# xuchang116/smCounter

Hardware: AMD Instinct MI355X
Metric: loci/sec at fixed read-depth x rpb (higher is better)
Workload: dtype u8/u32 scan + f64 posterior

## Files before the change

### include/smcounter_hip.h

```cpp
#ifndef SMCOUNTER_HIP_H
#define SMCOUNTER_HIP_H

#include <stdint.h>

#ifdef __cplusplus
extern "C" {
#endif

#define SMC_ABI_VERSION 11
#define SMC_MAX_ALLELES 64

#define SMC_OK 0
#define SMC_E_ARG (-1)
#define SMC_E_HIP (-2)
#define SMC_E_NOGPU (-3)
#define SMC_E_INPUT (-4)

#define SMC_ST_OK 0
#define SMC_ST_ZERO_COVERAGE 1
#define SMC_ST_DOWNSAMPLED 0x100
#define SMC_ST_BAD_INPUT 0x200
#define SMC_ST_UNDERFLOW 0x400

#define SMC_F_LM 0x001
// ... 307 lines not shown
int smc_spike_alleles(smc_ctx* ctx, const smc_dev_aln* d_aln, int64_t n_aln, const uint32_t* d_cig, const uint8_t* d_bq, int64_t n_pairs,
                      const smc_spike_variant* d_var, const smc_spike_variant* var_host, int32_t n_var, const uint64_t* d_idents,
                      int64_t n_bc, uint64_t seed, double mismatch_thr, const int32_t* d_nm, const int32_t* d_n_indel,
                      smc_dev_aln* d_aln_out, uint8_t* d_bq_out, uint32_t* d_stats, void* stream);
typedef struct smc_spike_indel_variant {
    int32_t pos0;
    uint8_t kind;
    uint8_t ref, alt;
    uint8_t pad;
    uint16_t len;
    uint16_t lead;
    uint32_t ins_off;
    uint64_t thr;
} smc_spike_indel_variant;
int smc_spike_indels(smc_ctx* ctx, const smc_dev_aln* d_aln, int64_t n_aln, const uint32_t* d_cig, int64_t n_cig_words, const uint8_t* d_bq,
                     int64_t n_pairs, const smc_spike_indel_variant* d_var, const smc_spike_indel_variant* var_host, int32_t n_var,
                     const uint8_t* d_ins, int64_t n_ins, const uint64_t* d_idents, int64_t n_bc, uint64_t seed, double mismatch_thr,
                     const int32_t* d_nm, const int32_t* d_n_indel, int64_t cap_pairs, int64_t cap_cig, smc_dev_aln* d_aln_out,
                     uint8_t* d_bq_out, uint32_t* d_cig_out, int32_t* d_nm_out, int32_t* d_n_indel_out, uint32_t* d_stats,
                     uint64_t* d_totals, void* stream);
#define SMC_SPIKE_MAX_COPIES 64
#define SMC_SPIKE_REP_MAX_TARGETS 32
int smc_spike_alleles_reps(smc_ctx* ctx, const smc_dev_aln* d_aln, int64_t n_aln, const uint32_t* d_cig, const uint8_t* d_bq, int64_t n_pairs,
                           const smc_spike_variant* d_var, const smc_spike_variant* var_host, int32_t n_var, const uint64_t* d_idents,
                           int64_t n_bc, const uint64_t* seeds, const uint64_t* thr, int32_t n_copies, double mismatch_thr,
                           const int32_t* d_nm, const int32_t* d_n_indel, uint8_t* d_aln_out, int64_t aln_stride, uint8_t* d_bq_out,
                           int64_t bq_stride, uint32_t* d_stats, void* stream);
int smc_spike_rep_counts(smc_ctx* ctx, const uint64_t* d_cov_ident, const uint32_t* d_cov_cnt, const uint32_t* d_cov_off,
                         const uint32_t* cov_off_host, const uint32_t* d_pos1, int32_t n_var, const uint64_t* d_seeds, int32_t n_reps,
                         const uint64_t* thr, int32_t n_targets, uint32_t* d_out, void* stream);
int smc_spike_depth_counts(smc_ctx* ctx, const uint64_t* d_cov_ident, const uint32_t* d_cov_cnt, const uint32_t* d_cov_off,
                           const uint32_t* cov_off_host, const uint32_t* d_pos1, int32_t n_var, const uint64_t* d_seeds, int32_t n_reps,
                           const uint64_t* thr, int32_t n_targets, const uint64_t* depth_thr, int32_t n_fracs, uint32_t* d_out, void* stream);
#define SMC_SPIKE_PHASE_MAX_MEMBERS 8
int smc_spike_phase_counts(smc_ctx* ctx, const uint64_t* d_joint_ident, const uint32_t* d_joint_cnt, const uint32_t* d_joint_off,
                           const uint32_t* joint_off_host, const uint32_t* d_set_m, const uint32_t* set_m_host, const uint32_t* d_cnt_off,
                           const uint32_t* d_pos1, int32_t n_sets, const uint64_t* d_seeds, int32_t n_reps, const uint64_t* thr,
                           int32_t n_targets, const uint64_t* depth_thr, int32_t n_fracs, uint32_t* d_out, void* stream);
int smc_spike_indels_reps(smc_ctx* ctx, const smc_dev_aln* d_aln, int64_t n_aln, const uint32_t* d_cig, int64_t n_cig_words, const uint8_t* d_bq,
                          int64_t n_pairs, const smc_spike_indel_variant* d_var, const smc_spike_indel_variant* var_host, int32_t n_var,
                          const uint8_t* d_ins, int64_t n_ins, const uint64_t* d_idents, int64_t n_bc, const uint64_t* seeds, const uint64_t* thr,
                          int32_t n_copies, double mismatch_thr, const int32_t* d_nm, const int32_t* d_n_indel, int64_t cap_pairs,
                          int64_t cap_cig, uint8_t* d_aln_out, int64_t aln_stride, uint8_t* d_bq_out, int64_t bq_stride, uint8_t* d_cig_out,
                          int64_t cig_stride, int32_t* d_nm_out, int32_t* d_n_indel_out, uint32_t* d_stats, uint64_t* d_totals, void* stream);
int smc_spike_indel_touch(smc_ctx* ctx, const smc_dev_aln* d_aln, int64_t n_aln, const uint32_t* d_cig, int64_t n_cig_words, int64_t n_pairs,
                          const smc_spike_indel_variant* d_var, const smc_spike_indel_variant* var_host, int32_t n_var, int64_t n_bc,
                          uint32_t* d_out, void* stream);
int smc_spike_indel_counts(smc_ctx* ctx, const uint64_t* d_cov_ident, const uint32_t* d_cov_cnt, const uint32_t* d_cov_off,
                           const uint32_t* cov_off_host, const uint32_t* d_pos1, int32_t n_var, const uint64_t* d_seeds, int32_t n_reps,
                           const uint64_t* thr, int32_t n_targets, const uint64_t* depth_thr, int32_t n_fracs, uint32_t* d_out, void* stream);
int smc_spike_indel_phase_counts(smc_ctx* ctx, const uint64_t* d_joint_ident, const uint32_t* d_joint_cnt, const uint32_t* d_joint_off,
                                 const uint32_t* joint_off_host, const uint32_t* d_set_m, const uint32_t* set_m_host, const uint32_t* d_cnt_off,
                                 const uint32_t* d_pos1, int32_t n_sets, const uint64_t* d_seeds, int32_t n_reps, const uint64_t* thr,
                                 int32_t n_targets, const uint64_t* depth_thr, int32_t n_fracs, uint32_t* d_out, void* stream);
int smc_spike_read_bits(smc_ctx* ctx, const smc_dev_aln* d_aln, int64_t n_aln, const uint32_t* d_cig, int64_t n_cig_words, const uint8_t* d_bq,
                        int64_t n_pairs, const smc_dev_locus* d_loc, int64_t n_loci, int32_t start0, const smc_af_variant* d_var,
                        const smc_af_variant* var_host, int32_t n_var, uint8_t* d_out, void* stream);
int smc_spike_rpb_counts(smc_ctx* ctx, const uint64_t* d_cov_ident, const uint32_t* d_cov_off, const uint32_t* cov_off_host,
                         const uint32_t* d_rec_off, const uint32_t* rec_off_host, const uint64_t* d_rec_name, const uint8_t* d_rec_flag,
                         int64_t n_rec, const uint32_t* d_pos1, int32_t n_var, const uint64_t* d_seeds, int32_t n_reps, const uint64_t* thr,
                         int32_t n_targets, const uint64_t* read_thr, int32_t n_read_thr, uint32_t* d_out, void* stream);
int smc_read_groups_counts_frac_seeds(smc_read_groups* g, const uint64_t* seeds, int32_t n_seeds, const uint64_t* bc_thr, int32_t n_frac,
                                      uint64_t* counts);
int smc_spike_grid_counts(smc_ctx* ctx, const uint64_t* d_cov_ident, const uint32_t* d_cov_off, const uint32_t* cov_off_host,
                          const uint32_t* d_rec_off, const uint32_t* rec_off_host, const uint64_t* d_rec_name, const uint8_t* d_rec_flag,
                          int64_t n_rec, const uint32_t* d_pos1, int32_t n_var, const uint64_t* d_seeds, int32_t n_reps, const uint64_t* thr,
                          int32_t n_targets, const uint64_t* bc_thr, int32_t n_fracs, const uint64_t* d_rd_thr, const uint64_t* rd_thr_host,
                          int32_t n_read_thr, uint32_t* d_out, void* stream);
int smc_spike_indel_read_bits(smc_ctx* ctx, const smc_dev_aln* d_aln, int64_t n_aln, const uint32_t* d_cig, int64_t n_cig_words,
                              const uint8_t* d_bq, int64_t n_pairs, const smc_dev_locus* d_loc, int64_t n_loci, int32_t start0,
                              const smc_spike_indel_variant* d_var, const smc_spike_indel_variant* var_host, int32_t n_var,
                              const uint8_t* d_ins, int64_t n_ins, uint8_t* d_out, void* stream);
int smc_spike_indel_rpb_counts(smc_ctx* ctx, const uint64_t* d_cov_ident, const uint32_t* d_cov_off, const uint32_t* cov_off_host,
                               const uint32_t* d_rec_off, const uint32_t* rec_off_host, const uint64_t* d_rec_name, const uint8_t* d_rec_flag,
                               int64_t n_rec, const uint32_t* d_pos1, int32_t n_var, const uint64_t* d_seeds, int32_t n_reps,
                               const uint64_t* thr, int32_t n_targets, const uint64_t* read_thr, int32_t n_read_thr, uint32_t* d_out,
                               void* stream);
int smc_spike_phase_rpb_counts(smc_ctx* ctx, const uint64_t* d_joint_ident, const uint32_t* d_joint_off, const uint32_t* joint_off_host,
                               const uint32_t* d_set_m, const uint32_t* set_m_host, const uint32_t* d_seg_base, const uint32_t* seg_base_host,
                               const uint32_t* d_rec_off, const uint32_t* rec_off_host, const uint64_t* d_rec_name, const uint8_t* d_rec_flag,
                               int64_t n_rec, const uint32_t* d_pos1, int32_t n_sets, const uint64_t* d_seeds, int32_t n_reps,
                               const uint64_t* thr, int32_t n_targets, const uint64_t* read_thr, int32_t n_read_thr, uint32_t* d_out,
                               void* stream);

typedef struct smc_scan_locus {
    uint32_t offset;
    uint32_t alt;
} smc_scan_locus;
typedef struct smc_scan_verdict {
    double pi;
    int32_t vmt;
    uint32_t mt_verdict;
} smc_scan_verdict;
#define SMC_SCAN_NOT 0u
#define SMC_SCAN_CALLED 1u
#define SMC_SCAN_HOST 2u
#define SMC_SCAN_MT_MASK 0x3FFFFFFFu
int smc_scan_detect(smc_ctx* ctx, const smc_row* d_rows, int32_t n_copies, int64_t n_loci, const smc_scan_locus* d_listed,
                    const smc_scan_locus* listed_host, int32_t n_listed, double thr, smc_scan_verdict* d_out, uint32_t* d_host_list,
                    uint32_t* d_n_host, void* stream);
#define SMC_SCAN_ID_NONE 0xFFFFFFFFu
#define SMC_SCAN_ID_HOST 0xFFFFFFFEu
int smc_scan_detect_keys(smc_ctx* ctx, const smc_row* d_rows, int32_t n_copies, int64_t n_loci, const smc_af_variant* d_var,
                         const smc_af_variant* var_host, int32_t n_listed, const uint8_t* d_ins, int64_t n_ins, const smc_dev_aln* d_aln,
                         int64_t aln_stride, const uint32_t* d_cig, int64_t cig_stride, const uint8_t* d_bq, int64_t bq_stride, int64_t n_aln,
                         int64_t cap_pairs, const uint32_t* d_x, int64_t x_stride, const uint32_t* d_xcount, int64_t xcount_stride,
                         int64_t xcap, double thr, uint32_t* d_alt_id, smc_scan_verdict* d_out, uint32_t* d_host_list, uint32_t* d_n_host,
                         void* stream);
#define SMC_F_REPT 0x0400u
#define SMC_F_REPS 0x0800u
#define SMC_F_SL 0x1000u
#define SMC_F_OTHER_REPEAT 0x2000u
#define SMC_SCAN_FLT_DEVICE_MASK 0x3FFu
#define SMC_SCAN_FLT_NAMES_MASK 0x3FFFu
#define SMC_SCAN_FLT_HOST 0x80000000u
int smc_scan_filter(smc_ctx* ctx, const smc_row* d_rows, int32_t n_copies, int64_t n_loci, const uint32_t* d_offsets,
                    const uint32_t* offsets_host, const uint32_t* d_gate, const uint32_t* gate_host, const uint32_t* d_always,
                    const uint32_t* always_host, int32_t n_listed, uint32_t* d_out, void* stream);
int smc_plan_info(const smc_plan* plan, int32_t* n_launches, int64_t* scratch_bytes);

int smc_plan_set_timing(smc_plan* plan, int slots);
int smc_plan_kernel_ms(smc_plan* plan, float* avg_ms, int32_t* n_samples, int64_t* n_loci, int64_t* n_reads);

int smc_plan_run(smc_plan* plan, const smc_params* params, const uint32_t* meta,
                 const uint32_t* umi, const uint32_t* frag, const uint32_t* dist,
                 const uint32_t* umi_start, smc_row* rows, void* stream);
int smc_plan_run_words(smc_plan* plan, const smc_params* params, const uint32_t* words, const uint32_t* umi_start,
                       smc_row* rows, void* stream);
int smc_plan_run_words16(smc_plan* plan, const smc_params* params, const uint16_t* words16, const uint32_t* umi_start,
                         smc_row* rows, void* stream);
int smc_pack_words(smc_plan* plan, const uint32_t* meta, const uint32_t* frag, uint32_t* words, void* stream);

int smc_call_batch_host(smc_ctx* ctx, const smc_params* params, const smc_locus* loci,
                        int64_t n_loci, const uint32_t* meta, const uint32_t* umi,
                        const uint32_t* frag, const uint32_t* dist, int64_t n_slots,
                        const uint32_t* umi_start, int64_t n_umi_start, smc_row* rows_out);

int smc_wire_row_size(void);
int smc_pack_rows(smc_ctx* ctx, const smc_row* rows, int64_t n, smc_wire_row* wire, void* stream);
int smc_unpack_rows(const smc_wire_row* wire, int64_t n, smc_row* rows);

typedef struct smc_build_in {
    const smc_dev_aln* aln; const uint32_t* cig;
    const uint8_t* bq;
    const smc_dev_locus* loc; const uint8_t* refseq;
    int32_t start0, n_loci, n_bc, n_pair;
    int32_t max_depth;
    int32_t n_aln;
    const smc_dev_locus* loc_host;
} smc_build_in;
int smc_build_max_depth(void);
int smc_build_set_timing(smc_ctx* ctx, int slots);
int smc_build_kernel_ms(smc_ctx* ctx, float* avg_ms, int32_t* n_samples);
int smc_build_planes(smc_ctx* ctx, const smc_params* params, const smc_build_in* in, uint32_t slot_base, uint32_t umi_base,
                     uint32_t* words, uint32_t* meta, uint32_t* umi, uint32_t* frag, uint32_t* dist, uint32_t* umi_start,
                     uint32_t* u_gid, uint32_t* u_finc, smc_locus* loci, uint32_t* xlist, uint32_t xcap, uint32_t* counters, void* stream);

int smc_build_planes_w16(smc_ctx* ctx, const smc_params* params, const smc_build_in* in, uint32_t slot_base, uint32_t umi_base,
                         uint16_t* words16, uint32_t* umi_start, uint32_t* u_gid, uint32_t* u_finc, smc_locus* loci,
                         uint32_t* xlist, uint32_t xcap, uint32_t* counters, void* stream);

#define SMC_LISTED_MAX_LOCI 64
#define SMC_LISTED_MAX_COPIES 1024
#define SMC_LISTED_UNFLAGGED 64u
#define SMC_LISTED_SHARED_ORDER 1
#define SMC_LISTED_DENSE_LOCUS 2
typedef struct smc_listed_copy {
    const smc_dev_aln* aln; const uint32_t* cig; const uint8_t* bq; const smc_dev_locus* loc;
    int32_t n_aln, n_bc, n_pair, reserved;
} smc_listed_copy;
int smc_build_listed(smc_ctx* ctx, const smc_params* params, const smc_listed_copy* d_copies, int32_t n_copies, int32_t flags,
                     int32_t start0, int32_t n_loci, const uint8_t* d_refseq, const uint32_t* offsets, const uint32_t* caps,
                     int32_t n_listed, int32_t word_bits, uint32_t slot_base, uint32_t umi_base, void* words, uint32_t* umi_start,
                     uint32_t* u_gid, uint32_t* u_finc, smc_locus* loci, uint32_t* xlist, uint32_t xcap, uint32_t* counters,
                     void* stream);

int smc_pool_trim(smc_ctx* ctx);

int smc_mem_alloc(smc_ctx* ctx, int64_t bytes, void** out);
void smc_mem_free(smc_ctx* ctx, void* p);
int smc_mem_alloc_best(smc_ctx* ctx, int64_t bytes, int tries, void** out, float* info);
int smc_mem_write_probe(smc_ctx* ctx, void* p, int64_t bytes, float* ms);
int smc_mem_alloc_host(smc_ctx* ctx, int64_t bytes, void** out);
void smc_mem_free_host(smc_ctx* ctx, void* p);
int smc_mem_h2d(smc_ctx* ctx, void* dst_device, const void* src_host, int64_t bytes);
int smc_mem_d2h(smc_ctx* ctx, void* dst_host, const void* src_device, int64_t bytes);
int smc_device_sync(smc_ctx* ctx);

int smc_event_create(void** ev);
int smc_event_record(void* ev, void* stream);
int smc_event_elapsed_ms(void* start, void* stop, float* ms);
void smc_event_destroy(void* ev);

#ifdef __cplusplus
}
#endif
#endif
```

### smcounter_amd/_lib.py

```python
from __future__ import annotations

import ctypes
import os

from . import abi

HERE = os.path.dirname(os.path.abspath(__file__))
LIB_PATH = os.environ.get("SMC_HIP_LIB") or os.path.join(HERE, "libsmcounter_hip.so")

SYMBOLS = ("smc_abi_version", "smc_last_error", "smc_row_size", "smc_locus_size", "smc_device_count",
           "smc_create", "smc_destroy", "smc_plan_create", "smc_plan_create_dev", "smc_plan_create_dev_spec", "smc_plan_spec_ok", "smc_plan_spec_counts", "smc_plan_hint_reset", "smc_philox_marks", "smc_philox4x32_10_host", "smc_select_alignments", "smc_select_alignments_keyed", "smc_select_alignments_copies", "smc_select_alignments_reads_copies", "smc_read_groups_create", "smc_read_groups_add", "smc_read_groups_finish",
           "smc_read_groups_masks", "smc_read_groups_kept", "smc_read_groups_status", "smc_read_groups_destroy",
           "smc_read_groups_counts_frac", "smc_read_groups_masks_grid", "smc_read_groups_kept_grid", "smc_lod_table", "smc_fisher_tables", "smc_lfact_values", "smc_allele_carriers", "smc_af_rep_masks", "smc_af_rep_counts", "smc_af_depth_masks", "smc_af_depth_counts", "smc_spike_alleles", "smc_spike_indels", "smc_spike_alleles_reps", "smc_spike_rep_counts", "smc_spike_depth_counts", "smc_spike_phase_counts", "smc_spike_indels_reps", "smc_spike_indel_touch", "smc_spike_indel_counts", "smc_spike_indel_phase_counts", "smc_spike_read_bits", "smc_spike_rpb_counts", "smc_spike_indel_read_bits", "smc_spike_indel_rpb_counts", "smc_spike_phase_rpb_counts", "smc_read_groups_counts_frac_seeds", "smc_spike_grid_counts", "smc_scan_detect", "smc_scan_detect_keys", "smc_scan_filter", "smc_plan_destroy", "smc_plan_info",
           "smc_plan_run", "smc_plan_run_words", "smc_plan_run_words16", "smc_pack_words", "smc_plan_set_timing", "smc_plan_kernel_ms", "smc_call_batch_host", "smc_event_create", "smc_event_record",
           "smc_event_elapsed_ms", "smc_event_destroy", "smc_class_table", "smc_wire_row_size", "smc_pack_rows", "smc_unpack_rows",
           "smc_build_planes", "smc_build_planes_w16", "smc_build_listed", "smc_build_max_depth", "smc_build_set_timing", "smc_build_kernel_ms", "smc_mem_alloc", "smc_mem_alloc_best", "smc_mem_write_probe", "smc_mem_free", "smc_mem_h2d", "smc_mem_d2h",
           "smc_mem_alloc_host", "smc_mem_free_host", "smc_pool_trim",
           "smc_device_sync")


class SmcError(RuntimeError):
    pass


def exp_env(name: str, default=None):
    on = os.environ.get("SMC_EXPERIMENTAL", "0") not in ("", "0")
    return os.environ.get(name, default) if on else default


_LIB = None


def load(with_torch: bool = True):
    global _LIB
    if _LIB is not None:
        return _LIB
    if not os.path.exists(LIB_PATH):
        try:
            from . import build
            build.build_hip()
        except Exception as e:
            raise SmcError("HIP library missing: %s and it could not be built (%s) - run `python -c 'import "
                           "__graft_entry__ as g; g.build()'`; there is no CPU fallback" % (LIB_PATH, e))
    if with_torch:
        try:
            import torch
        except ImportError:
            pass
    L = ctypes.CDLL(LIB_PATH)
    vp, i32, i64 = ctypes.c_void_p, ctypes.c_int32, ctypes.c_int64
    L.smc_abi_version.restype = ctypes.c_int
    L.smc_last_error.restype = ctypes.c_char_p
    L.smc_row_size.restype = ctypes.c_int
    L.smc_locus_size.restype = ctypes.c_int
    L.smc_device_count.restype = ctypes.c_int
    L.smc_create.argtypes = [ctypes.c_int, ctypes.POINTER(vp)]
    L.smc_destroy.argtypes = [vp]
    L.smc_destroy.restype = None
    L.smc_plan_create.argtypes = [vp, vp, i64, ctypes.POINTER(vp)]
    L.smc_plan_create_dev.argtypes = [vp, vp, i64, vp, ctypes.POINTER(vp)]
    L.smc_plan_create_dev_spec.argtypes = [vp, ctypes.POINTER(abi.SmcParams), vp, i64, vp, ctypes.POINTER(vp)]
    L.smc_plan_spec_ok.argtypes = [vp, ctypes.POINTER(ctypes.c_int)]
    L.smc_plan_spec_counts.argtypes = [vp, ctypes.POINTER(i64), ctypes.POINTER(i64), ctypes.POINTER(i64)]
    L.smc_plan_hint_reset.argtypes = [vp]
    L.smc_philox_marks.argtypes = [vp, ctypes.POINTER(abi.SmcParams), vp, i64, vp, vp, ctypes.c_int, vp, vp, vp, ctypes.c_uint64, vp, vp]
    L.smc_philox4x32_10_host.argtypes = [vp, vp, vp]
    L.smc_philox4x32_10_host.restype = None
    L.smc_select_alignments.argtypes = [vp, vp, i64, vp, i64, i32, vp, vp, i64, ctypes.c_uint64, ctypes.c_double, vp, vp, vp, vp, vp]
    L.smc_select_alignments_keyed.argtypes = [vp, vp, i64, vp, i64, i32, i32, i64, i64, vp, vp, i64, ctypes.c_uint64, ctypes.c_double, vp, vp, vp, vp, vp]
    L.smc_select_alignments_copies.argtypes = [vp, vp, i64, i32, i64, vp, i64, i32, vp, i64, vp, vp, i32, vp, vp, vp, vp, vp]
    L.smc_select_alignments_reads_copies.argtypes = [vp, vp, i64, i32, i64, vp, i64, i32, i64, i64, vp, i64, i64, i32, i64, vp, vp, vp, vp, vp]
    L.smc_read_groups_create.argtypes = [vp, ctypes.POINTER(vp)]
    L.smc_read_groups_add.argtypes = [vp, vp, i64, i64]
    L.smc_read_groups_finish.argtypes = [vp, vp]
    L.smc_read_groups_masks.argtypes = [vp, vp, i64, ctypes.c_uint64, vp, i32, vp, vp]
    L.smc_read_groups_kept.argtypes = [vp, ctypes.c_uint64, vp, i32, vp]
    L.smc_read_groups_status.argtypes = [vp, ctypes.POINTER(ctypes.c_uint32)]
    L.smc_read_groups_counts_frac.argtypes = [vp, ctypes.c_uint64, vp, i32, vp]
    L.smc_read_groups_masks_grid.argtypes = [vp, vp, i64, ctypes.c_uint64, vp, vp, i32, vp, vp]
    L.smc_read_groups_kept_grid.argtypes = [vp, ctypes.c_uint64, vp, vp, i32, vp]
    L.smc_lod_table.argtypes = [vp, ctypes.c_int, ctypes.c_int, vp, vp]
    L.smc_fisher_tables.argtypes = [vp, vp, i64, vp, vp]
    L.smc_lfact_values.argtypes = [vp, vp, i64, vp]
    L.smc_allele_carriers.argtypes = [vp, vp, i64, vp, vp, vp, i64, i32, i64, vp, vp, i32, vp, i64, vp, vp, vp, vp]
    L.smc_af_rep_masks.argtypes = [vp, vp, i64, vp, vp, vp, vp, i64, i32, vp, i32, vp, i64, vp, vp]
    L.smc_af_rep_counts.argtypes = [vp, vp, vp, vp, vp, i32, vp, vp, vp, vp, i64, i32, vp, i32, vp, vp]
    L.smc_af_depth_masks.argtypes = [vp, vp, i64, vp, vp, vp, vp, i64, i32, vp, i32, vp, i32, vp, i64, vp, vp]
    L.smc_af_depth_counts.argtypes = [vp, vp, vp, vp, vp, i32, vp, vp, vp, vp, i64, i32, vp, i32, vp, i32, vp, vp]
    L.smc_spike_alleles.argtypes = [vp, vp, i64, vp, vp, i64, vp, vp, i32, vp, i64, ctypes.c_uint64, ctypes.c_double, vp, vp, vp, vp, vp, vp]
    L.smc_spike_indels.argtypes = [vp, vp, i64, vp, i64, vp, i64, vp, vp, i32, vp, i64, vp, i64, ctypes.c_uint64, ctypes.c_double, vp, vp, i64, i64,
                                   vp, vp, vp, vp, vp, vp, vp, vp]
    L.smc_spike_alleles_reps.argtypes = [vp, vp, i64, vp, vp, i64, vp, vp, i32, vp, i64, vp, vp, i32, ctypes.c_double, vp, vp, vp, i64, vp, i64, vp, vp]
    L.smc_spike_rep_counts.argtypes = [vp, vp, vp, vp, vp, vp, i32, vp, i32, vp, i32, vp, vp]
    L.smc_spike_depth_counts.argtypes = [vp, vp, vp, vp, vp, vp, i32, vp, i32, vp, i32, vp, i32, vp, vp]
    L.smc_spike_phase_counts.argtypes = [vp, vp, vp, vp, vp, vp, vp, vp, vp, i32, vp, i32, vp, i32, vp, i32, vp, vp]
    L.smc_spike_indels_reps.argtypes = [vp, vp, i64, vp, i64, vp, i64, vp, vp, i32, vp, i64, vp, i64, vp, vp, i32, ctypes.c_double, vp, vp, i64, i64,
                                        vp, i64, vp, i64, vp, i64, vp, vp, vp, vp, vp]
    L.smc_spike_indel_touch.argtypes = [vp, vp, i64, vp, i64, i64, vp, vp, i32, i64, vp, vp]
    L.smc_spike_indel_counts.argtypes = [vp, vp, vp, vp, vp, vp, i32, vp, i32, vp, i32, vp, i32, vp, vp]
    L.smc_spike_indel_phase_counts.argtypes = L.smc_spike_phase_counts.argtypes
    L.smc_spike_read_bits.argtypes = [vp, vp, i64, vp, i64, vp, i64, vp, i64, i32, vp, vp, i32, vp, vp]
    L.smc_spike_rpb_counts.argtypes = [vp, vp, vp, vp, vp, vp, vp, vp, i64, vp, i32, vp, i32, vp, i32, vp, i32, vp, vp]
    L.smc_read_groups_counts_frac_seeds.argtypes = [vp, vp, i32, vp, i32, vp]
    L.smc_spike_grid_counts.argtypes = [vp, vp, vp, vp, vp, vp, vp, vp, i64, vp, i32, vp, i32, vp, i32, vp, i32, vp, vp, i32, vp, vp]
    L.smc_spike_indel_read_bits.argtypes = [vp, vp, i64, vp, i64, vp, i64, vp, i64, i32, vp, vp, i32, vp, i64, vp, vp]
    L.smc_spike_indel_rpb_counts.argtypes = L.smc_spike_rpb_counts.argtypes
    L.smc_spike_phase_rpb_counts.argtypes = [vp, vp, vp, vp, vp, vp, vp, vp, vp, vp, vp, vp, i64, vp, i32, vp, i32, vp, i32, vp, i32, vp, vp]
    L.smc_scan_detect.argtypes = [vp, vp, i32, i64, vp, vp, i32, ctypes.c_double, vp, vp, vp, vp]
    L.smc_scan_detect_keys.argtypes = [vp, vp, i32, i64, vp, vp, i32, vp, i64, vp, i64, vp, i64, vp, i64, i64, i64, vp, i64, vp, i64, i64,
                                       ctypes.c_double, vp, vp, vp, vp, vp]
    L.smc_scan_filter.argtypes = [vp, vp, i32, i64, vp, vp, vp, vp, vp, vp, i32, vp, vp]
    L.smc_read_groups_destroy.argtypes = [vp]
    L.smc_read_groups_destroy.restype = None
    L.smc_plan_destroy.argtypes = [vp]
    L.smc_plan_destroy.restype = None
    L.smc_plan_info.argtypes = [vp, ctypes.POINTER(i32), ctypes.POINTER(i64)]
    L.smc_plan_run.argtypes = [vp, ctypes.POINTER(abi.SmcParams), vp, vp, vp, vp, vp, vp, vp]
    L.smc_plan_run_words.argtypes = [vp, ctypes.POINTER(abi.SmcParams), vp, vp, vp, vp]
    L.smc_plan_run_words16.argtypes = [vp, ctypes.POINTER(abi.SmcParams), vp, vp, vp, vp]
    L.smc_pack_words.argtypes = [vp, vp, vp, vp, vp]
    L.smc_plan_set_timing.argtypes = [vp, ctypes.c_int]
    L.smc_plan_kernel_ms.argtypes = [vp, ctypes.POINTER(ctypes.c_float), ctypes.POINTER(i32), ctypes.POINTER(i64),
                                     ctypes.POINTER(i64)]
    L.smc_call_batch_host.argtypes = [vp, ctypes.POINTER(abi.SmcParams), vp, i64, vp, vp, vp, vp, i64, vp, i64, vp]
    L.smc_wire_row_size.restype = ctypes.c_int
    L.smc_pack_rows.argtypes = [vp, vp, i64, vp, vp]
    L.smc_unpack_rows.argtypes = [vp, i64, vp]
    L.smc_mem_alloc.argtypes = [vp, i64, ctypes.POINTER(vp)]
    L.smc_mem_alloc_best.argtypes = [vp, i64, ctypes.c_int, ctypes.POINTER(vp), ctypes.POINTER(ctypes.c_float)]
    L.smc_mem_write_probe.argtypes = [vp, vp, i64, ctypes.POINTER(ctypes.c_float)]
    L.smc_mem_free.argtypes = [vp, vp]
    L.smc_mem_free.restype = None
    L.smc_mem_alloc_host.argtypes = [vp, i64, ctypes.POINTER(vp)]
    L.smc_mem_free_host.argtypes = [vp, vp]
    L.smc_mem_free_host.restype = None
    L.smc_mem_h2d.argtypes = [vp, vp, vp, i64]
    L.smc_mem_d2h.argtypes = [vp, vp, vp, i64]
    L.smc_device_sync.argtypes = [vp]
    L.smc_pool_trim.argtypes = [vp]
    L.smc_build_max_depth.restype = ctypes.c_int
    L.smc_build_set_timing.argtypes = [vp, ctypes.c_int]
    L.smc_build_kernel_ms.argtypes = [vp, ctypes.POINTER(ctypes.c_float), ctypes.POINTER(ctypes.c_int32)]
    L.smc_build_planes.argtypes = [vp, ctypes.POINTER(abi.SmcParams), ctypes.POINTER(abi.SmcBuildIn), ctypes.c_uint32,
                                   ctypes.c_uint32, vp, vp, vp, vp, vp, vp, vp, vp, vp, vp, ctypes.c_uint32, vp, vp]
    L.smc_build_planes_w16.argtypes = [vp, ctypes.POINTER(abi.SmcParams), ctypes.POINTER(abi.SmcBuildIn), ctypes.c_uint32,
                                       ctypes.c_uint32, vp, vp, vp, vp, vp, vp, ctypes.c_uint32, vp, vp]
    L.smc_build_listed.argtypes = [vp, ctypes.POINTER(abi.SmcParams), vp, i32, i32, i32, i32, vp, vp, vp, i32, i32, ctypes.c_uint32, ctypes.c_uint32,
                                   vp, vp, vp, vp, vp, vp, ctypes.c_uint32, vp, vp]
    L.smc_event_create.argtypes = [ctypes.POINTER(vp)]
    L.smc_event_record.argtypes = [vp, vp]
    L.smc_event_elapsed_ms.argtypes = [vp, vp, ctypes.POINTER(ctypes.c_float)]
    L.smc_event_destroy.argtypes = [vp]
    L.smc_event_destroy.restype = None
    if L.smc_abi_version() != 11:
        raise SmcError("ABI version mismatch")
    if L.smc_row_size() != abi.ROW_DTYPE.itemsize or L.smc_locus_size() != 32 or L.smc_wire_row_size() != abi.WIRE_DTYPE.itemsize:
        raise SmcError("struct layout mismatch between include/smcounter_hip.h and smcounter_amd/abi.py")
    _LIB = L
    return L


def check(rc: int, what: str):
    if rc != 0:
        raise SmcError("%s failed (%d): %s" % (what, rc, load().smc_last_error().decode()))
```

### smcounter_amd/csrc/bp_masks.h

```cpp
#pragma once
#include <stdint.h>
#if defined(__HIPCC__)
#define BP_HD __host__ __device__ __forceinline__
#else
#define BP_HD static inline
#endif
BP_HD uint32_t bp_heads(uint32_t C, uint32_t S, bool carried) {
    const uint32_t K1 = S, K2 = K1 & (K1 << 1), K4 = K2 & (K2 << 2), K8 = K4 & (K4 << 4), K16 = K8 & (K8 << 8);
    uint32_t V = C;
    V |= (V << 1) & K1; V |= (V << 2) & K2; V |= (V << 4) & K4; V |= (V << 8) & K8; V |= (V << 16) & K16;
    uint32_t H = C & ~((V << 1) & S);
    const uint32_t t = ~(S | 1u), G0 = t ? (t & (0u - t)) - 1u : 0xFFFFFFFFu;
    if (carried) H &= ~G0;
    return H;
}
```

### smcounter_amd/csrc/host_abi.inc

```
static const char* exp_env(const char* name) {
    const char* const xv = getenv("SMC_EXPERIMENTAL");
    const bool on = xv && *xv && strcmp(xv, "0") != 0;
    const char* v = getenv(name);
    if (v && !on) {
        static bool told = false;
        if (!told) { told = true; fprintf(stderr, "smcounter_hip: %s is set but SMC_EXPERIMENTAL is not: experiment switches are ignored\n", name); }
        return nullptr;
    }
    return v;
}
static thread_local std::string g_err;
static int fail(int code, const std::string& msg) { g_err = msg; return code; }
#define HIPCHK(x)                                                                                   \
    do {                                                                                            \
        hipError_t e_ = (x);                                                                        \
        if (e_ != hipSuccess)                                                                       \
            return fail(SMC_E_HIP, std::string(#x) + ": " + hipGetErrorString(e_));                 \
    } while (0)

struct smc_ctx {
    int device;
    void* bp_scratch = nullptr;
    size_t bp_bytes = 0;
    hipEvent_t bp_done_ev = nullptr;
    void* sel_scratch = nullptr;
    size_t sel_bytes = 0;
    void* lod_scratch = nullptr;
    size_t lod_bytes = 0;
    void* af_scratch = nullptr;
    size_t af_bytes = 0;
    void* spi_scratch = nullptr;
    size_t spi_bytes = 0;
    void* bl_scratch = nullptr;
    size_t bl_bytes = 0;
    hipEvent_t bl_done_ev = nullptr;
    void* chk_scratch = nullptr;
    size_t chk_bytes = 0;
    struct SegStage { void* host = nullptr; size_t cap = 0; hipEvent_t ev = nullptr; bool used = false; };
    SegStage seg_stage[4];
    int seg_next = 0;
    std::vector<hipEvent_t> bp_ev0, bp_ev1;
    int64_t bp_timed = 0;
    std::vector<std::pair<size_t, void*>> plan_pool;
    struct PendingFree { hipEvent_t ev; std::vector<std::pair<size_t, void*>> blocks; };
    std::vector<PendingFree> plan_pending;
    void* plan_stats = nullptr;
    void* plan_stats_host = nullptr;
    bool plan_stats_clean = false;
    hipEvent_t plan_fill_ev = nullptr;
    void* plan_deep = nullptr;
    size_t plan_deep_cap = 0;
    bool hint_ok = false;
    int64_t hint_loci = 0;
    PlanStats hint_stats;
    uint32_t* d_spec_fail = nullptr;
    std::vector<void*> spec_host_free;
    int64_t spec_made = 0, spec_failed = 0, spec_exact = 0;
    struct VmmBlock { void* va; size_t total; std::vector<hipMemGenericAllocationHandle_t> handles; };
    std::vector<VmmBlock> vmm;
    std::mutex vmm_mu;
    double* lut;
    double* simple;
    double* pcr;
    double* lfact = nullptr;
    int max_lds;
    int n_cu = 256;
};

static int grow_scratch(void*& ptr, size_t& have, size_t need, size_t want, const char* who, const hipStream_t* sync) {
    if (need <= have) return SMC_OK;
    if (sync) { const hipStream_t st = *sync; HIPCHK(hipStreamSynchronize(st)); }
    (void)hipFree(ptr);
    ptr = nullptr; have = 0;
    hipError_t e = hipMalloc(&ptr, want);
    if (e != hipSuccess) return fail(SMC_E_HIP, std::string(who) + ": " + std::to_string(want) + " bytes of scratch: " + hipGetErrorString(e));
    have = want;
    return SMC_OK;
}

static size_t plan_size_class(size_t bytes) {
    if (bytes > ((size_t)256 << 20)) return (bytes + ((size_t)64 << 20) - 1) & ~(((size_t)64 << 20) - 1);
    size_t c = 256;
    while (c < bytes) c <<= 1;
    return c;
}
#define SMC_POOL_BLOCKS 64
#define SMC_POOL_BYTES ((size_t)8 << 30)
static void plan_pool_put(smc_ctx* ctx, size_t cls, void* p) {
    if (cls > ((size_t)1 << 30)) { (void)hipFree(p); return; }
    size_t held = cls;
    for (auto& b : ctx->plan_pool) held += b.first;
    while (!ctx->plan_pool.empty() && (ctx->plan_pool.size() >= SMC_POOL_BLOCKS || held > SMC_POOL_BYTES)) {
        held -= ctx->plan_pool.front().first;
        (void)hipFree(ctx->plan_pool.front().second);
        ctx->plan_pool.erase(ctx->plan_pool.begin());
    }
    ctx->plan_pool.emplace_back(cls, p);
}
static void plan_pool_collect(smc_ctx* ctx, bool all) {
    for (size_t i = 0; i < ctx->plan_pending.size();) {
        auto& q = ctx->plan_pending[i];
        if (all || ctx->plan_pending.size() > 16) (void)hipEventSynchronize(q.ev);
        else if (hipEventQuery(q.ev) != hipSuccess) { ++i; continue; }
        for (auto& b : q.blocks) plan_pool_put(ctx, b.first, b.second);
        (void)hipEventDestroy(q.ev);
        ctx->plan_pending.erase(ctx->plan_pending.begin() + (long)i);
    }
}
static hipError_t plan_alloc(smc_ctx* ctx, void** out, size_t bytes) {
    const size_t cls = plan_size_class(bytes);
    plan_pool_collect(ctx, false);
    hipError_t e = hipErrorOutOfMemory;
    for (size_t i = 0; i < ctx->plan_pool.size(); ++i)
        if (ctx->plan_pool[i].first == cls) { *out = ctx->plan_pool[i].second; ctx->plan_pool.erase(ctx->plan_pool.begin() + (long)i); e = hipSuccess; break; }
    if (e != hipSuccess) e = hipMalloc(out, cls);
    if (e == hipSuccess) if (const char* v = exp_env("SMC_PLAN_POISON")) {
        (void)hipDeviceSynchronize();
        e = hipMemset(*out, atoi(v) & 0xFF, cls);
        if (e == hipSuccess) e = hipDeviceSynchronize();
    }
    return e;
}

static size_t host_hdr_bytes(int a_cap) {
    return sizeof(Hdr) + (size_t)a_cap * SMC_NT * 4 + (size_t)a_cap * 8 + (size_t)a_cap * 4 + (size_t)a_cap * 4 + 128 * 8 + 32 * 8;
}
static size_t whole_locus_lds(const smc_locus& L, int a_cap) {
    return host_hdr_bytes(a_cap) + 4 * (((size_t)L.n_reads + 3) / 4 + 2) + 9 * (size_t)L.n_umi + 32;
}
static size_t bin_lds_bytes(int a_cap, size_t fcap, size_t ucap) { return (host_hdr_bytes(a_cap) + 4 * fcap + 9 * ucap + 32 + 255) & ~(size_t)255; }

#ifndef SMC_R0
#define SMC_R0 4096
#endif
#ifndef SMC_R1
#define SMC_R1 8192
#endif
#ifndef SMC_R2
#define SMC_R2 12288
#endif
#ifndef SMC_R3
#define SMC_R3 24576
#endif
#ifndef SMC_DEEP_BLOCK
#define SMC_DEEP_BLOCK 512
#endif
#ifndef SMC_DEEP_FCAP
#define SMC_DEEP_FCAP 5376
#endif
#ifndef SMC_DEEP_UCAP
#define SMC_DEEP_UCAP 2560
#endif
#ifndef SMC_DEEP_PART_READS
#define SMC_DEEP_PART_READS 20480
#endif
#define SMC_CLS_DEEP 4

struct Bin {
    int cls;
    int a_cap = 8;
    int fcap = 0, ucap = 0;
    size_t lds_bytes = 0;
    std::vector<int> order;
    std::vector<V2Part> parts;
    size_t n_parts = 0;
    V2Part* d_parts = nullptr;
    smc_locus* d_desc = nullptr;
    size_t desc_bytes = 0;
    int64_t* d_flags_off = nullptr;
    uint32_t* d_flags = nullptr;
    uint32_t* d_acc = nullptr;
    size_t acc_bytes = 0, flags_bytes = 0, parts_bytes = 0, foff_bytes = 0;
    int64_t reads = 0;
    const uint32_t* d_launch_n = nullptr;
};

struct smc_plan {
    smc_ctx* ctx;
    int64_t n_loci;
    smc_locus* d_loci = nullptr;
    bool own_loci = true;
    uint32_t* d_flt_list = nullptr;
    uint16_t fp = 0;
    int64_t need_quads = 0;
    hipEvent_t done_ev = nullptr;
    bool flt_clean = false;
    int flt_parity = 0;
    size_t loci_bytes = 0, flt_bytes = 0, words_bytes = 0;
    uint32_t* d_words = nullptr;
    std::vector<Bin> bins;
    int timing = 0, dom_bin = -1;
    int64_t dom_loci = 0, dom_reads = 0;
    std::vector<hipEvent_t> ev0, ev1;
    int64_t n_timed = 0;
    bool spec = false;
// ... 2029 lines not shown
    if (!p || !prm) return fail(SMC_E_ARG, "smc_plan_run: NULL argument");
    if (p->n_loci == 0) return SMC_OK;
    if (p->spec) return fail(SMC_E_ARG, "smc_plan_run: a plan made by smc_plan_create_dev_spec runs read words (smc_plan_run_words / _words16), not raw-field planes");
    (void)umi; (void)dist;
    if (!meta || !frag || !umi_start || !rows) return fail(SMC_E_ARG, "smc_plan_run: NULL device pointer");
    HIPCHK(hipSetDevice(p->ctx->device));
    if (!p->d_words) { p->words_bytes = 16 * (size_t)std::max<int64_t>(1, p->need_quads); HIPCHK(plan_alloc(p->ctx, (void**)&p->d_words, p->words_bytes)); }
    int rc = smc_pack_words(p, meta, frag, p->d_words, stream);
    if (rc) return rc;
    return smc_plan_run_words(p, prm, p->d_words, umi_start, rows, stream);
}

int smc_call_batch_host(smc_ctx* ctx, const smc_params* prm, const smc_locus* loci, int64_t n_loci, const uint32_t* meta,
                        const uint32_t* umi, const uint32_t* frag, const uint32_t* dist, int64_t n_slots,
                        const uint32_t* umi_start, int64_t n_umi_start, smc_row* rows_out) {
    if (!ctx || !prm || (n_loci && (!loci || !rows_out))) return fail(SMC_E_ARG, "smc_call_batch_host: NULL argument");
    if (n_loci == 0) return SMC_OK;
    for (int64_t l = 0; l < n_loci; ++l) {
        const smc_locus& L = loci[l];
        if (L.n_reads < 0 || L.n_umi < 0 || 4ll * L.read_off4 + L.n_reads > n_slots ||
            (int64_t)L.umi_off + L.n_umi + 1 > n_umi_start)
            return fail(SMC_E_INPUT, "smc_call_batch_host: locus " + std::to_string(l) + " points outside the planes / umi_start");
    }
    HIPCHK(hipSetDevice(ctx->device));
    smc_plan* plan = nullptr;
    int rc = smc_plan_create(ctx, loci, n_loci, &plan);
    if (rc) return rc;
    uint32_t* d[5] = {nullptr, nullptr, nullptr, nullptr, nullptr};
    const uint32_t* h[5] = {meta, umi, frag, dist, umi_start};
    const int64_t hn[5] = {n_slots, n_slots, n_slots, n_slots, n_umi_start};
    smc_row* d_rows = nullptr;

    auto cleanup = [&]() {
        for (auto q : d) (void)hipFree(q);
        (void)hipFree(d_rows);
        smc_plan_destroy(plan);
    };
    (void)umi; (void)dist;
    for (int k = 0; k < 5; ++k) {
        if (k == 1 || k == 3) continue;
        hipError_t e = hipMalloc(&d[k], sizeof(uint32_t) * (size_t)(hn[k] > 0 ? hn[k] : 1));
        if (e == hipSuccess && hn[k] > 0) e = hipMemcpy(d[k], h[k], sizeof(uint32_t) * (size_t)hn[k], hipMemcpyHostToDevice);
        if (e != hipSuccess) { cleanup(); return fail(SMC_E_HIP, std::string("plane upload: ") + hipGetErrorString(e)); }
    }
    hipError_t e = hipMalloc(&d_rows, sizeof(smc_row) * (size_t)n_loci);
    if (e != hipSuccess) { cleanup(); return fail(SMC_E_HIP, std::string("rows alloc: ") + hipGetErrorString(e)); }
    rc = smc_plan_run(plan, prm, d[0], d[1], d[2], d[3], d[4], d_rows, nullptr);
    if (rc == SMC_OK) {
        e = hipDeviceSynchronize();
        if (e == hipSuccess) e = hipMemcpy(rows_out, d_rows, sizeof(smc_row) * (size_t)n_loci, hipMemcpyDeviceToHost);
        if (e != hipSuccess) rc = fail(SMC_E_HIP, std::string("run/download: ") + hipGetErrorString(e));
    }
    cleanup();
    return rc;
}

int smc_build_max_depth(void) { return (1 << 24) - 1; }

static int build_planes_impl(smc_ctx* ctx, const smc_params* prm, const smc_build_in* in, uint32_t slot_base, uint32_t umi_base,
                             uint32_t* words, bool w16, uint32_t* meta, uint32_t* umi, uint32_t* frag, uint32_t* dist, uint32_t* umi_start,
                             uint32_t* u_gid, uint32_t* u_finc, smc_locus* loci, uint32_t* xlist, uint32_t xcap, uint32_t* counters, void* stream);
int smc_build_planes(smc_ctx* ctx, const smc_params* prm, const smc_build_in* in, uint32_t slot_base, uint32_t umi_base,
                     uint32_t* words, uint32_t* meta, uint32_t* umi, uint32_t* frag, uint32_t* dist, uint32_t* umi_start,
                     uint32_t* u_gid, uint32_t* u_finc, smc_locus* loci, uint32_t* xlist, uint32_t xcap, uint32_t* counters, void* stream) {
    return build_planes_impl(ctx, prm, in, slot_base, umi_base, words, false, meta, umi, frag, dist, umi_start, u_gid, u_finc, loci, xlist, xcap, counters, stream);
}
int smc_build_planes_w16(smc_ctx* ctx, const smc_params* prm, const smc_build_in* in, uint32_t slot_base, uint32_t umi_base,
                         uint16_t* words16, uint32_t* umi_start, uint32_t* u_gid, uint32_t* u_finc, smc_locus* loci,
                         uint32_t* xlist, uint32_t xcap, uint32_t* counters, void* stream) {
    if (!words16) return fail(SMC_E_ARG, "smc_build_planes_w16: NULL device pointer");
    if (prm && (prm->min_bq < 0 || prm->min_bq > 63)) return fail(SMC_E_INPUT, "smc_build_planes_w16: minBQ " + std::to_string(prm->min_bq) + " has no room in a 16-bit read word (0 .. 63)");
    return build_planes_impl(ctx, prm, in, slot_base, umi_base, (uint32_t*)words16, true, nullptr, nullptr, nullptr, nullptr, umi_start, u_gid, u_finc, loci, xlist, xcap, counters, stream);
}
static int build_planes_impl(smc_ctx* ctx, const smc_params* prm, const smc_build_in* in, uint32_t slot_base, uint32_t umi_base,
                             uint32_t* words, bool w16, uint32_t* meta, uint32_t* umi, uint32_t* frag, uint32_t* dist, uint32_t* umi_start,
                             uint32_t* u_gid, uint32_t* u_finc, smc_locus* loci, uint32_t* xlist, uint32_t xcap, uint32_t* counters, void* stream) {
    if (!ctx || !prm || !in || !counters) return fail(SMC_E_ARG, "smc_build_planes: NULL argument");
    if (in->n_loci <= 0) return SMC_OK;
    if (!in->aln || !in->cig || !in->bq || !in->loc || !in->refseq || !(words || (meta && frag)) || !umi_start ||
        !u_gid || !u_finc || !loci || !xlist) return fail(SMC_E_ARG, "smc_build_planes: NULL device pointer");
    if (in->max_depth < 0 || in->max_depth > smc_build_max_depth())
        return fail(SMC_E_INPUT, "smc_build_planes: a locus of " + std::to_string(in->max_depth) + " reads (limit " + std::to_string(smc_build_max_depth()) + ")");
    HIPCHK(hipSetDevice(ctx->device));
    hipStream_t st = (hipStream_t)stream;
    const int n_loci = in->n_loci, n_tiles = (n_loci + BP_TILE - 1) / BP_TILE;
    std::vector<smc_dev_locus> loc_copy;
    const smc_dev_locus* lh = in->loc_host;
    if (!lh) {
        loc_copy.resize((size_t)n_loci);
        HIPCHK(hipMemcpy(loc_copy.data(), in->loc, sizeof(smc_dev_locus) * (size_t)n_loci, hipMemcpyDeviceToHost));
        lh = loc_copy.data();
    }
    int tiles_per_seg = 1;
    for (int t = 0; t < n_tiles && tiles_per_seg == 1; ++t) {
        const int l0 = t * BP_TILE, l1 = std::min(n_loci, l0 + BP_TILE) - 1;
        if (lh[l1].w1 > lh[l0].w0 && lh[l1].w1 - lh[l0].w0 > BP_LSORT_MAX) tiles_per_seg = BP_SEG_TILES_DEEP;
    }
    { const char* v = exp_env("SMC_BP_SEG_TILES"); if (v && atoi(v) >= 1) tiles_per_seg = atoi(v); }
    const int seg_loci = tiles_per_seg * BP_TILE, n_seg = (n_loci + seg_loci - 1) / seg_loci;
    uint64_t ntot = 0, work = 0, reads = 0;
    std::vector<uint32_t> seg_cnt((size_t)n_seg), seg_tiles((size_t)n_seg);
    for (int s = 0; s < n_seg; ++s) {
        const int l0 = s * seg_loci, l1 = std::min(n_loci, l0 + seg_loci) - 1;
        const uint32_t w0 = lh[l0].w0, w1 = std::max(w0, lh[l1].w1);
        if (in->n_aln >= 0 && (int64_t)w1 > (int64_t)in->n_aln)
            return fail(SMC_E_INPUT, "smc_build_planes: locus window beyond the run's " + std::to_string(in->n_aln) + " alignments");
        seg_cnt[(size_t)s] = w1 - w0; seg_tiles[(size_t)s] = (uint32_t)((l1 - l0) / BP_TILE + 1);
        ntot += w1 - w0; work += (uint64_t)(w1 - w0) * seg_tiles[(size_t)s];
    }
    const bool tile_lists = tiles_per_seg > 1 && !exp_env("SMC_BP_NO_TILE_LISTS");
    std::vector<uint32_t> wcnt;
    uint64_t ntot_w = 0;
    int nch = 1;
    if (tile_lists) {
        wcnt.resize((size_t)n_tiles);
        for (int t = 0; t < n_tiles; ++t) {
            const int l0 = t * BP_TILE, l1 = std::min(n_loci, l0 + BP_TILE) - 1;
            const uint32_t w0 = lh[l0].w0, w1 = std::max(w0, lh[l1].w1);
            wcnt[(size_t)t] = w1 - w0; ntot_w += w1 - w0;
        }
        for (int s = 0; s < n_seg; ++s) nch = std::max(nch, (int)((seg_cnt[(size_t)s] + BP_TL_CH - 1) / BP_TL_CH));
        work = ntot_w;
        if (ntot_w >= (1ull << 31)) return fail(SMC_E_INPUT, "smc_build_planes: run too large (entries of the tiles' lists " + std::to_string(ntot_w) + ")");
    }
    for (int l = 0; l < n_loci; ++l) reads += lh[l].n;
    int64_t n_aln = in->n_aln;
    if (n_aln < 0) { n_aln = 0; for (int l = 0; l < n_loci; ++l) n_aln = std::max<int64_t>(n_aln, lh[l].w1); }
    if (ntot >= (1ull << 31) || reads >= (1ull << 32)) return fail(SMC_E_INPUT, "smc_build_planes: run too large (sorted entries " + std::to_string(ntot) + ", reads " + std::to_string(reads) + ")");
    uint32_t part = (uint32_t)std::min<uint64_t>(4096, std::max<uint64_t>(256, (work / 81920 + 63) / 64 * 64));
    { const char* v = exp_env("SMC_BP_PART"); if (v && atoi(v) >= 64) part = (uint32_t)std::min(4096, atoi(v)) / 64u * 64u; }
    int rs_maxblk = BP_RS_MAXBLK;
    { const char* v = exp_env("SMC_BP_RS_MAXBLK"); if (v && atoi(v) > 0) rs_maxblk = atoi(v); }
    const uint32_t max_blk = (uint32_t)std::max(1, rs_maxblk / n_seg);
    uint64_t total_blk = 0, total_parts = 0, total_cparts = 0;
    for (int s = 0; s < n_seg; ++s) {
        total_blk += bp_seg_blocks(seg_cnt[(size_t)s], max_blk);
        if (tile_lists) continue;
        total_parts += (uint64_t)((seg_cnt[(size_t)s] + BP_SUB - 1) / BP_SUB) * seg_tiles[(size_t)s];
        total_cparts += (uint64_t)((seg_cnt[(size_t)s] + part - 1) / part) * seg_tiles[(size_t)s];
    }
    if (tile_lists)
        for (int t = 0; t < n_tiles; ++t) {
            total_parts += (uint64_t)((wcnt[(size_t)t] + BP_SUB - 1) / BP_SUB);
            total_cparts += (uint64_t)((wcnt[(size_t)t] + part - 1) / part);
        }
    if (total_parts >= (1ull << 31)) return fail(SMC_E_INPUT, "smc_build_planes: too many (tile, part) wavefronts");
    int bc_bits = 1, pair_bits = 1;
    while (bc_bits < 32 && (1ll << bc_bits) < (int64_t)std::max(1, in->n_bc)) ++bc_bits;
    while (pair_bits < 32 && (1ll << pair_bits) < (int64_t)std::max(1, in->n_pair)) ++pair_bits;
    const int passes = (bc_bits + pair_bits + 7) / 8;
    const uint32_t xraw_cap = (uint32_t)std::min<uint64_t>(1u << 28, reads / 32 + 65536);
    size_t off = 0;
    auto carve = [&](size_t bytes) { const size_t o = off; off += (bytes + 255) & ~(size_t)255; return o; };
    const size_t o_seg = carve(sizeof(BpSeg) * (size_t)n_seg);
    const size_t o_wseg = carve(tile_lists ? sizeof(BpSeg) * (size_t)n_tiles : 0), o_sorted2 = carve(tile_lists ? 4 * (size_t)ntot_w : 0),
                 o_tc = carve(tile_lists ? 4 * (size_t)n_tiles * (size_t)nch : 0);
    const size_t o_k0 = carve(8 * (size_t)ntot), o_k1 = carve(8 * (size_t)ntot), o_v0 = carve(4 * (size_t)ntot), o_v1 = carve(4 * (size_t)ntot);
    const size_t o_hist = carve(4 * 256 * (size_t)total_blk), o_dtot = carve(4 * 256 * (size_t)n_seg);
    const size_t o_cnt = carve(768 * (size_t)total_cparts), o_cntp = carve(256 * (size_t)total_parts), o_pstate = carve(16 * (size_t)total_parts);
    const uint32_t n_rblk = (uint32_t)((std::max<int64_t>(1, n_aln) + 255) / 256);
    const size_t lin_cap = (size_t)std::min<uint64_t>(0xFFFF0000ull, ((uint64_t)1 << 20) + 24ull * (uint64_t)std::max<int64_t>(1, n_aln));
    const size_t o_rows = carve(32 * (size_t)std::max<int64_t>(1, n_aln)), o_need = carve(4 * (size_t)std::max<int64_t>(1, n_aln));
    const size_t o_bsum = carve(128 * BP_NCUR + 256), o_lin = carve(2 * lin_cap + 256);
    const uint32_t glist_stride = 256u * ((n_rblk + BP_NCUR - 1) / BP_NCUR) + 64u;
    const size_t o_glist = carve(4 * (size_t)glist_stride * BP_NCUR), o_k8 = carve(8 * (size_t)std::max<int64_t>(1, n_aln));
    const size_t o_zero = off;
    const size_t o_xcnt = carve(4 * (size_t)n_loci), o_tcnt = carve(4 * ((size_t)n_tiles + 1)), o_tcur = carve(4 * (size_t)n_tiles), o_xn = carve(4);
    const size_t o_zend = off;
    const size_t o_xraw = carve(4 * BP_XW * (size_t)xraw_cap), o_gidx = carve(4 * ((size_t)xraw_cap + 4)), o_gidx2 = carve(4 * ((size_t)xraw_cap + 4));
    if (int rc = grow_scratch(ctx->bp_scratch, ctx->bp_bytes, off, off + off / 8, "smc_build_planes", &st)) return rc;
    char* sc = (char*)ctx->bp_scratch;
    if (ctx->bp_done_ev) HIPCHK(hipStreamWaitEvent(st, ctx->bp_done_ev, 0));
    if (const char* v = exp_env("SMC_BP_POISON_SCRATCH")) HIPCHK(hipMemsetAsync(sc, atoi(v) & 0xFF, ctx->bp_bytes, st));
    if (!total_parts) {
        HIPCHK(hipMemsetAsync(sc + o_zero, 0, o_zend - o_zero, st));
        HIPCHK(hipMemsetAsync(counters, 0, 8, st));
    }
    BpArgs A;
    A.aln = in->aln; A.cig = in->cig; A.bq = in->bq; A.loc = in->loc; A.refseq = in->refseq;
    A.start0 = in->start0; A.n_loci = n_loci; A.n_seg = n_seg; A.part = (int32_t)part; A.seg_tiles = tiles_per_seg;
    A.min_bq = prm->min_bq; A.min_mq = prm->min_mq; A.primer_dist = prm->primer_dist; A.ds = prm->ds;
    A.fp = (uint32_t)smc_param_fingerprint(prm->min_bq, prm->min_mq, prm->mismatch_thr, prm->primer_dist) << SMC_LF_FP_SHIFT;
    A.slot_base = slot_base; A.umi_base = umi_base;
    { const char* v = exp_env("SMC_BP_XCD_ROT"); A.xcd_rot = v ? (uint32_t)atoi(v) & 7u : 0u; }
    { const char* v = exp_env("SMC_BP_XCD_GROUP"); if (v && atoi(v) > 0) A.xcd_rot |= (uint32_t)atoi(v) << 8; }
    A.words = words; A.w16 = w16 ? 1u : 0u; A.meta = meta; A.umi = umi; A.frag = frag; A.dist = dist; A.umi_start = umi_start; A.u_gid = u_gid; A.u_finc = u_finc;
    A.loci = loci;
    BpSeg* d_seg = (BpSeg*)(sc + o_seg);
    A.seg = d_seg;
    A.cnt = (uint32_t*)(sc + o_cnt); A.cntp = (uint32_t*)(sc + o_cntp); A.pstate = (uint32_t*)(sc + o_pstate);
    A.xraw = (uint32_t*)(sc + o_xraw); A.xraw_cap = xraw_cap; A.xraw_n = (uint32_t*)(sc + o_xn);
    A.xcnt = (uint32_t*)(sc + o_xcnt); A.tcnt = (uint32_t*)(sc + o_tcnt); A.tcur = (uint32_t*)(sc + o_tcur); A.gidx = (uint32_t*)(sc + o_gidx); A.gidx2 = (uint32_t*)(sc + o_gidx2);
    A.xlist = xlist; A.xcap = xcap; A.xcount = counters; A.status = counters + 1;
    BpSeg* d_wseg = (BpSeg*)(sc + o_wseg);
    if (tile_lists || (in->loc_host && !exp_env("SMC_BP_SEGTAB_DEV"))) {
        smc_ctx::SegStage& SG = ctx->seg_stage[ctx->seg_next];
        ctx->seg_next = (ctx->seg_next + 1) % 4;
        if (SG.used) HIPCHK(hipEventSynchronize(SG.ev));
        const size_t n_stage = (size_t)n_seg + (tile_lists ? (size_t)n_tiles : 0);
        if (SG.cap < sizeof(BpSeg) * n_stage) {
            if (SG.host) (void)hipHostFree(SG.host);
            SG.host = nullptr; SG.cap = 0;
            const size_t want = std::max<size_t>(4096, sizeof(BpSeg) * n_stage * 2);
            HIPCHK(hipHostMalloc(&SG.host, want, hipHostMallocDefault));
            SG.cap = want;
        }
        if (!SG.ev) HIPCHK(hipEventCreateWithFlags(&SG.ev, hipEventDisableTiming));
        BpSeg* hs = (BpSeg*)SG.host;
        uint32_t off_run = 0, part_run = 0, blk_run = 0, cpart_run = 0;
        for (int sgi = 0; sgi < n_seg; ++sgi) {
            BpSeg S{};
            const int l0 = sgi * seg_loci, l1 = std::min(n_loci, l0 + seg_loci) - 1;
            S.w0 = lh[l0].w0;
            S.w1 = std::max(S.w0, lh[l1].w1);
            const uint32_t cnt = S.w1 - S.w0;
            S.n_tiles = (uint32_t)((l1 - l0) / BP_TILE + 1);
            S.ppt = (cnt + BP_SUB - 1) / BP_SUB;
            S.cppt = (cnt + part - 1) / part;
            S.n_blk = bp_seg_blocks(cnt, max_blk);
            S.off = off_run; S.part_base = part_run; S.blk_base = blk_run; S.cpart_base = cpart_run;
            off_run += cnt; part_run += S.ppt * S.n_tiles; blk_run += S.n_blk; cpart_run += S.cppt * S.n_tiles;
            hs[(size_t)sgi] = S;
        }
        HIPCHK(hipMemcpyAsync(d_seg, hs, sizeof(BpSeg) * (size_t)n_seg, hipMemcpyHostToDevice, st));
        if (tile_lists) {
            BpSeg* hw = hs + n_seg;
            uint32_t woff = 0, wpart = 0, wcpart = 0;
            for (int t = 0; t < n_tiles; ++t) {
                BpSeg S{};
                const int l0 = t * BP_TILE, l1 = std::min(n_loci, l0 + BP_TILE) - 1;
                S.w0 = lh[l0].w0; S.w1 = std::max(S.w0, lh[l1].w1);
                const uint32_t cnt = S.w1 - S.w0;
                S.n_tiles = 1u; S.ppt = (cnt + BP_SUB - 1) / BP_SUB; S.cppt = (cnt + part - 1) / part; S.n_blk = 0u;
                S.off = woff; S.part_base = wpart; S.blk_base = 0u; S.cpart_base = wcpart;
                woff += cnt; wpart += S.ppt; wcpart += S.cppt;
                hw[(size_t)t] = S;
            }
            HIPCHK(hipMemcpyAsync(d_wseg, hw, sizeof(BpSeg) * (size_t)n_tiles, hipMemcpyHostToDevice, st));
        }
        HIPCHK(hipEventRecord(SG.ev, st));
        SG.used = true;
    } else
        hipLaunchKernelGGL(k_bp_segtab, dim3(1), dim3(1024), 0, st, in->loc, n_loci, n_seg, seg_loci, part, max_blk, d_seg);
    HIPCHK(hipGetLastError());
    const bool raw = meta || umi || frag || dist;
    BpRow* d_rows = (BpRow*)(sc + o_rows);
    uint8_t* d_lin = (uint8_t*)(sc + o_lin);
    uint2* d_k8 = (uint2*)(sc + o_k8);
    uint32_t* d_bsum = (uint32_t*)(sc + o_bsum);
    uint32_t* d_glist = (uint32_t*)(sc + o_glist);
    if (total_parts) {
        hipLaunchKernelGGL(k_bp_zero_words, dim3(8), dim3(256), 0, st, d_bsum, 32u * BP_NCUR);
        hipLaunchKernelGGL(k_bp_rows_write, dim3(n_rblk), dim3(256), 0, st, A, (uint32_t)n_aln, d_bsum, d_glist, glist_stride, d_rows, (uint32_t)lin_cap, raw ? 1 : 0, d_k8,
                           (uint32_t*)(sc + o_zero), (uint32_t)((o_zend - o_zero) / 4), counters);
    }
    unsigned long long* kb[2] = {(unsigned long long*)(sc + o_k0), (unsigned long long*)(sc + o_k1)};
    uint32_t* vb[2] = {(uint32_t*)(sc + o_v0), (uint32_t*)(sc + o_v1)};
    uint32_t* d_hist = (uint32_t*)(sc + o_hist);
    int cur = 0;
    bool any_small = false, any_mid = false;
    for (int s = 0; s < n_seg; ++s) {
        any_small |= seg_cnt[(size_t)s] > 0 && seg_cnt[(size_t)s] <= BP_LSORT_MAX;
        any_mid |= seg_cnt[(size_t)s] > BP_SORT_LDS_MAX && seg_cnt[(size_t)s] <= BP_LSORT_MAX;
    }
    if (any_small) {
        const bool big = any_mid && !exp_env("SMC_BP_SORT_SMALL");
        bool any_le = false;
        for (int s = 0; s < n_seg; ++s) any_le |= seg_cnt[(size_t)s] > 0 && seg_cnt[(size_t)s] <= BP_SORT_LDS_MAX;
        if (any_le || !big)
            hipLaunchKernelGGL((k_bp_sort_seg<BP_SORT_REG, BP_SORT_WAVES_SMALL, false>), dim3((unsigned)n_seg), dim3(64 * BP_SORT_WAVES_SMALL), 0, st, d_seg, d_k8, pair_bits, passes, kb[0], kb[1], vb[0], vb[1],
                               0u, big ? (uint32_t)BP_SORT_LDS_MAX : (uint32_t)BP_LSORT_MAX);
        if (big)
            hipLaunchKernelGGL((k_bp_sort_seg<BP_SORT_REG_BIG, BP_SORT_WAVES, true>), dim3((unsigned)n_seg), dim3(64 * BP_SORT_WAVES), 0, st, d_seg, d_k8, pair_bits, passes, kb[0], kb[1], vb[0], vb[1],
                               (uint32_t)BP_SORT_LDS_MAX, (uint32_t)BP_LSORT_MAX);
    }
    if (total_blk) {
        for (int ps = 0; ps < passes; ++ps) {
            const int shift = 8 * ps;
            if (ps == 0) hipLaunchKernelGGL(k_bp_hist<true>, dim3((unsigned)total_blk), dim3(64), 0, st, d_seg, n_seg, d_k8, pair_bits, kb[0], vb[0], shift, d_hist);
            else hipLaunchKernelGGL(k_bp_hist<false>, dim3((unsigned)total_blk), dim3(64), 0, st, d_seg, n_seg, d_k8, pair_bits, kb[cur], vb[cur], shift, d_hist);
            hipLaunchKernelGGL(k_bp_rowscan, dim3(256u * (unsigned)n_seg), dim3(64), 0, st, d_seg, d_hist, (uint32_t*)(sc + o_dtot));
            hipLaunchKernelGGL(k_bp_scatter, dim3((unsigned)total_blk), dim3(64), 0, st, d_seg, n_seg, kb[cur], vb[cur], kb[cur ^ 1], vb[cur ^ 1], shift, d_hist,
                               (const uint32_t*)(sc + o_dtot));
            cur ^= 1;
        }
        HIPCHK(hipGetLastError());
    }
    A.sorted = vb[passes & 1];
    if (tile_lists && total_parts) {
        uint32_t* d_tc = (uint32_t*)(sc + o_tc);
        uint32_t* d_sorted2 = (uint32_t*)(sc + o_sorted2);
        const unsigned tgrid = (unsigned)((size_t)n_tiles * (size_t)nch);
        hipLaunchKernelGGL(k_bp_tile_count, dim3(tgrid), dim3(256), 0, st, d_seg, tiles_per_seg, d_wseg, n_tiles, nch, A.sorted, d_tc);
        hipLaunchKernelGGL(k_bp_tile_scatter, dim3(tgrid), dim3(256), 0, st, d_seg, tiles_per_seg, d_wseg, n_tiles, nch, A.sorted, d_tc, d_sorted2);
        A.sorted = d_sorted2; A.seg = d_wseg; A.n_seg = n_tiles; A.seg_tiles = 1;
    }
    if (total_parts) {
        int64_t lin_grid = 2048;
        { const char* v = exp_env("SMC_BP_LIN_GRID"); if (v && atoi(v) > 0) lin_grid = atoi(v); }
        const int64_t lin_wgs = std::max<int64_t>(BP_NCUR, std::min<int64_t>(lin_grid, (n_aln + 15) / 16) / BP_NCUR * BP_NCUR);
        if (!raw) hipLaunchKernelGGL(k_bp_lin, dim3((unsigned)lin_wgs), dim3(256), 0, st, A, d_glist, glist_stride, d_bsum, d_rows, d_lin);
        hipLaunchKernelGGL(k_bp_count, dim3((unsigned)total_cparts), dim3(64), 0, st, A);
    }
    hipLaunchKernelGGL(k_bp_scan_tiles, dim3((unsigned)n_tiles), dim3(256), 0, st, A);
    if (total_parts) {
        const bool timed = !ctx->bp_ev0.empty();
        const size_t ev = timed ? (size_t)(ctx->bp_timed % (int64_t)ctx->bp_ev0.size()) : 0;
        if (timed) HIPCHK(hipEventRecord(ctx->bp_ev0[ev], st));
        size_t lds_pad = 0;
        { const char* v = exp_env("SMC_BP_LDS_PAD"); if (v) lds_pad = (size_t)std::max(0, atoi(v)); }
        if (raw) hipLaunchKernelGGL((k_bp_emit2<true, false>), dim3((unsigned)total_parts), dim3(64), lds_pad, st, A, d_rows, d_lin);
        else if (w16) hipLaunchKernelGGL((k_bp_emit2<false, true>), dim3((unsigned)total_parts), dim3(64), lds_pad, st, A, d_rows, d_lin);
        else hipLaunchKernelGGL((k_bp_emit2<false, false>), dim3((unsigned)total_parts), dim3(64), lds_pad, st, A, d_rows, d_lin);
        if (timed) { HIPCHK(hipEventRecord(ctx->bp_ev1[ev], st)); ctx->bp_timed++; }
        hipLaunchKernelGGL(k_bp_scan, dim3(1), dim3(1024), 0, st, A.tcnt, (uint32_t)n_tiles + 1u, (const uint32_t*)nullptr);
        hipLaunchKernelGGL(k_bp_xgroup, dim3(256), dim3(256), 0, st, A);
        hipLaunchKernelGGL(k_bp_xfix2, dim3((unsigned)n_tiles), dim3(64), 0, st, A);
        hipLaunchKernelGGL(k_bp_xfix, dim3((unsigned)n_tiles), dim3(64 * BP_XF_WAVES), 0, st, A);
    }
    HIPCHK(hipGetLastError());
    if (!ctx->bp_done_ev) HIPCHK(hipEventCreateWithFlags(&ctx->bp_done_ev, hipEventDisableTiming));
    HIPCHK(hipEventRecord(ctx->bp_done_ev, st));
    return SMC_OK;
}

int smc_build_listed(smc_ctx* ctx, const smc_params* prm, const smc_listed_copy* d_copies, int32_t n_copies, int32_t flags,
                     int32_t start0, int32_t n_loci, const uint8_t* d_refseq, const uint32_t* offsets, const uint32_t* caps,
                     int32_t n_listed, int32_t word_bits, uint32_t slot_base, uint32_t umi_base, void* words, uint32_t* umi_start,
                     uint32_t* u_gid, uint32_t* u_finc, smc_locus* loci, uint32_t* xlist, uint32_t xcap, uint32_t* counters,
                     void* stream) {
    const std::string who = "smc_build_listed";
    static_assert(sizeof(smc_listed_copy) == 48, "smc_build_listed's copy record");
    static_assert(SMC_LISTED_MAX_LOCI == BL_MAX_LOCI && SMC_LISTED_MAX_COPIES == BL_MAX_COPIES && SMC_LISTED_UNFLAGGED == BL_ST_UNFLAGGED, "smc_build_listed's limits");
    if (!ctx || !prm) return fail(SMC_E_ARG, who + ": NULL argument");
    if (n_copies < 0 || n_copies > SMC_LISTED_MAX_COPIES)
        return fail(SMC_E_INPUT, who + ": " + std::to_string(n_copies) + " copies, 0 .. " + std::to_string(SMC_LISTED_MAX_COPIES) + " expected");
    if (n_listed < 0 || n_listed > SMC_LISTED_MAX_LOCI)
        return fail(SMC_E_INPUT, who + ": " + std::to_string(n_listed) + " listed loci, 0 .. " + std::to_string(SMC_LISTED_MAX_LOCI) + " expected");
    if (word_bits != 16 && word_bits != 32) return fail(SMC_E_INPUT, who + ": read words of " + std::to_string(word_bits) + " bits, 16 or 32 expected");
    if (word_bits == 16 && (prm->min_bq < 0 || prm->min_bq > 63))
        return fail(SMC_E_INPUT, who + ": minBQ " + std::to_string(prm->min_bq) + " has no room in a 16-bit read word (0 .. 63)");
    if (n_loci < 0) return fail(SMC_E_INPUT, who + ": a run of " + std::to_string(n_loci) + " loci");
    if (flags & ~(SMC_LISTED_SHARED_ORDER | SMC_LISTED_DENSE_LOCUS)) return fail(SMC_E_INPUT, who + ": flags " + std::to_string(flags) + ", bits 0 and 1 expected");
    const bool shared_order = (flags & SMC_LISTED_SHARED_ORDER) != 0;
    if (!n_copies) return SMC_OK;
    if (!d_copies || !counters) return fail(SMC_E_ARG, who + ": NULL device pointer");
    if (n_listed && (!offsets || !caps)) return fail(SMC_E_ARG, who + ": NULL argument with " + std::to_string(n_listed) + " listed loci");
    if (n_listed && (!d_refseq || !words || !umi_start || !u_gid || !u_finc || !loci || !xlist)) return fail(SMC_E_ARG, who + ": NULL device pointer");
    if (slot_base & 3u) return fail(SMC_E_INPUT, who + ": slot_base " + std::to_string(slot_base) + " is not on a 4-read boundary");
    BlArgs A{};
    uint64_t stride = 0;
    uint32_t cap_max = 0;
    for (int32_t g = 0; g < n_listed; ++g) {
        if ((int64_t)offsets[g] >= (int64_t)n_loci)
            return fail(SMC_E_INPUT, who + ": listed locus " + std::to_string(g) + " names offset " + std::to_string(offsets[g]) + " of " + std::to_string(n_loci));
        if (g && offsets[g] <= offsets[g - 1]) return fail(SMC_E_INPUT, who + ": the listed offsets do not ascend at entry " + std::to_string(g));
        if ((caps[g] & 3u) || caps[g] > (uint32_t)smc_build_max_depth() + 1u)
            return fail(SMC_E_INPUT, who + ": listed locus " + std::to_string(g) + " has a capacity of " + std::to_string(caps[g]) +
                                     " slots (a multiple of 4, at most " + std::to_string(smc_build_max_depth() + 1) + ")");
        A.off[g] = offsets[g]; A.capoff[g] = (uint32_t)stride;
        stride += caps[g];
        cap_max = std::max(cap_max, caps[g]);
    }
    A.capoff[n_listed] = (uint32_t)stride;
    const uint64_t G = (uint64_t)n_listed, B = (uint64_t)n_copies;
    if ((uint64_t)slot_base + B * stride >= (1ull << 32) || (uint64_t)umi_base + B * (stride + G) + 1ull >= (1ull << 32))
        return fail(SMC_E_INPUT, who + ": " + std::to_string(n_copies) + " copies of " + std::to_string(stride) + " slots: 2^32 slots or more");
    HIPCHK(hipSetDevice(ctx->device));
    hipStream_t st = (hipStream_t)stream;
    const uint64_t Bo = shared_order ? 1ull : B;
    size_t off = 0;
    auto carve = [&](size_t bytes) { const size_t o = off; off += (bytes + 255) & ~(size_t)255; return o; };
    const size_t o_k0 = carve(8 * Bo * stride), o_k1 = carve(8 * Bo * stride), o_v0 = carve(4 * Bo * stride), o_v1 = carve(4 * Bo * stride);
    const size_t o_ord = carve(4 * Bo * stride), o_hi = carve(4 * Bo * stride), o_meta = carve(16 * Bo * G);
    const size_t o_cstat = carve(4 * B), o_st = carve(4 * B * G), o_nx = carve(4 * B * G), o_xtmp = carve(20 * (size_t)BL_XMAX * B * G);
    if (int rc = grow_scratch(ctx->bl_scratch, ctx->bl_bytes, off, off + off / 8, who.c_str(), &st)) return rc;
    if (ctx->bl_done_ev) HIPCHK(hipStreamWaitEvent(st, ctx->bl_done_ev, 0));
    char* sc = (char*)ctx->bl_scratch;
    A.copies = d_copies; A.refseq = d_refseq;
    A.n_copies = n_copies; A.n_listed = n_listed; A.shared = shared_order ? 1 : 0; A.dense = (flags & SMC_LISTED_DENSE_LOCUS) ? 1 : 0; A.start0 = start0;
    A.min_bq = prm->min_bq; A.min_mq = prm->min_mq; A.primer_dist = prm->primer_dist; A.ds = prm->ds;
    A.fp = (uint32_t)smc_param_fingerprint(prm->min_bq, prm->min_mq, prm->mismatch_thr, prm->primer_dist) << SMC_LF_FP_SHIFT;
    A.w16 = word_bits == 16 ? 1u : 0u; A.slot_base = slot_base; A.umi_base = umi_base; A.stride = (uint32_t)stride;
    A.words = words; A.umi_start = umi_start; A.u_gid = u_gid; A.u_finc = u_finc; A.loci = loci; A.xlist = xlist; A.xcap = xcap; A.counters = counters;
    A.key[0] = (unsigned long long*)(sc + o_k0); A.key[1] = (unsigned long long*)(sc + o_k1);
    A.val[0] = (uint32_t*)(sc + o_v0); A.val[1] = (uint32_t*)(sc + o_v1);
    A.order = (uint32_t*)(sc + o_ord); A.hinfo = (uint32_t*)(sc + o_hi); A.meta = (uint32_t*)(sc + o_meta);
    A.cstat = (uint32_t*)(sc + o_cstat); A.st = (uint32_t*)(sc + o_st); A.nx = (uint32_t*)(sc + o_nx); A.xtmp = (uint32_t*)(sc + o_xtmp);
    hipLaunchKernelGGL(k_bl_check, dim3((unsigned)n_copies), dim3(256), 0, st, A);
    if (n_listed) {
        hipLaunchKernelGGL(k_bl_sort, dim3((unsigned)n_listed, (unsigned)Bo), dim3(64 * BL_SORT_WAVES), 0, st, A);
        if (cap_max) hipLaunchKernelGGL(k_bl_words, dim3((cap_max + 255u) / 256u, (unsigned)n_listed, (unsigned)n_copies), dim3(256), 0, st, A);
        hipLaunchKernelGGL(k_bl_finish, dim3((unsigned)n_listed, (unsigned)n_copies), dim3(256), 0, st, A);
    }
    hipLaunchKernelGGL(k_bl_gather, dim3((unsigned)n_copies), dim3(64), 0, st, A);
    HIPCHK(hipGetLastError());
    if (!ctx->bl_done_ev) HIPCHK(hipEventCreateWithFlags(&ctx->bl_done_ev, hipEventDisableTiming));
    HIPCHK(hipEventRecord(ctx->bl_done_ev, st));
    return SMC_OK;
}

int smc_build_set_timing(smc_ctx* ctx, int slots) {
    if (!ctx || slots < 0) return fail(SMC_E_ARG, "smc_build_set_timing: bad argument");
    HIPCHK(hipSetDevice(ctx->device));
    for (auto e : ctx->bp_ev0) (void)hipEventDestroy(e);
    for (auto e : ctx->bp_ev1) (void)hipEventDestroy(e);
    ctx->bp_ev0.assign((size_t)slots, nullptr);
    ctx->bp_ev1.assign((size_t)slots, nullptr);
    for (int k = 0; k < slots; ++k) { HIPCHK(hipEventCreate(&ctx->bp_ev0[(size_t)k])); HIPCHK(hipEventCreate(&ctx->bp_ev1[(size_t)k])); }
    ctx->bp_timed = 0;
    return SMC_OK;
}
int smc_build_kernel_ms(smc_ctx* ctx, float* avg_ms, int32_t* n_samples) {
    if (!ctx || !avg_ms) return fail(SMC_E_ARG, "smc_build_kernel_ms: NULL argument");
    const int64_t ns = std::min<int64_t>(ctx->bp_timed, (int64_t)ctx->bp_ev0.size());
    if (ns <= 0) return fail(SMC_E_ARG, "smc_build_kernel_ms: no timed run (smc_build_set_timing(ctx, slots) then smc_build_planes)");
    double tot = 0;
    for (int64_t k = 0; k < ns; ++k) {
        float ms = 0;
        HIPCHK(hipEventSynchronize(ctx->bp_ev1[(size_t)k]));
        HIPCHK(hipEventElapsedTime(&ms, ctx->bp_ev0[(size_t)k], ctx->bp_ev1[(size_t)k]));
        tot += ms;
    }
    *avg_ms = (float)(tot / ns);
    if (n_samples) *n_samples = (int32_t)ns;
    return SMC_OK;
}

int smc_wire_row_size(void) { return (int)sizeof(smc_wire_row); }

int smc_pack_rows(smc_ctx* ctx, const smc_row* rows, int64_t n, smc_wire_row* wire, void* stream) {
    if (!ctx || n < 0 || (n > 0 && (!rows || !wire))) return fail(SMC_E_ARG, "smc_pack_rows: bad argument");
    if (n == 0) return SMC_OK;
    HIPCHK(hipSetDevice(ctx->device));
    const long long words = (long long)n * WIRE_WORDS;
    hipLaunchKernelGGL(k_pack_rows, dim3((unsigned)((words + 255) / 256)), dim3(256), 0, (hipStream_t)stream, rows, (uint32_t*)wire, words);
    HIPCHK(hipGetLastError());
    return SMC_OK;
}

int smc_unpack_rows(const smc_wire_row* wire, int64_t n, smc_row* rows) {
    if (n < 0 || (n > 0 && (!wire || !rows))) return fail(SMC_E_ARG, "smc_unpack_rows: bad argument");
    for (int64_t i = 0; i < n; ++i) {
        const smc_wire_row& W = wire[i];
        smc_row& R = rows[i];
        memset(&R, 0, sizeof R);
        R.status = (int32_t)(W.status & 0xFFFFu);
        R.biallelic = (W.status & SMC_WIRE_BIALLELIC) ? 1 : 0;
        R.cvg = W.cvg; R.all_frag = W.all_frag; R.all_mt = W.all_mt; R.used_frag = W.used_frag; R.used_mt = W.used_mt;
        R.mt3 = W.mt3; R.mt5 = W.mt5; R.mt7 = W.mt7; R.mt10 = W.mt10;
        R.max_allele = R.second_allele = -1;
        for (int a = 0; a < 4; ++a) { R.dp[a] = W.dp[a]; R.umt[a] = W.umt[a]; R.vsm[a] = W.vsm[a]; R.pi[a] = W.pi[a]; }
        for (int c = 0; c < 2; ++c) {
            const smc_wire_cand& wc = W.cand[c];
            smc_cand& C = R.cand[c];
            C.allele = wc.allele;
            C.flt = wc.flags & SMC_WIRE_FLT_MASK;
            C.flt_applied = (wc.flags & SMC_WIRE_FLT_APPLIED) ? 1 : 0;
            C.vmf_lt_099 = (wc.flags & SMC_WIRE_VMF_LT_099) ? 1 : 0;
            C.vdp = wc.vdp; C.vmt = wc.vmt; C.vsm = wc.vsm; C.pi = wc.pi;
            C.p_sb = C.p_r1 = C.p_r2 = C.p_pr = NAN;
        }
    }
    return SMC_OK;
}

int smc_pool_trim(smc_ctx* ctx) {
    if (!ctx) return fail(SMC_E_ARG, "smc_pool_trim: NULL context");
    HIPCHK(hipSetDevice(ctx->device));
    plan_pool_collect(ctx, true);
    for (auto& b : ctx->plan_pool) (void)hipFree(b.second);
    ctx->plan_pool.clear();
    return SMC_OK;
}

#ifndef SMC_VMM_CHUNK_MB
#define SMC_VMM_CHUNK_MB 64
#endif
#ifndef SMC_VMM_MIN_MB
#define SMC_VMM_MIN_MB 256
#endif
static hipError_t vmm_alloc(smc_ctx* ctx, size_t bytes, size_t chunk, void** out) {
    hipMemAllocationProp prop = {};
    prop.type = hipMemAllocationTypePinned; prop.location.type = hipMemLocationTypeDevice; prop.location.id = ctx->device;
    size_t gran = 0;
    hipError_t e = hipMemGetAllocationGranularity(&gran, &prop, hipMemAllocationGranularityRecommended);
    if (e != hipSuccess) return e;
    if (gran == 0) gran = 4096;
    chunk = (chunk + gran - 1) / gran * gran;
    const size_t total = (bytes + chunk - 1) / chunk * chunk;
    void* va = nullptr;
    e = hipMemAddressReserve(&va, total, (size_t)2 << 20, nullptr, 0);
    if (e != hipSuccess) return e;
    size_t mapped = 0;
    std::vector<hipMemGenericAllocationHandle_t> handles;
    const bool early_release = exp_env("SMC_VMM_EARLY_RELEASE") != nullptr;
    for (; mapped < total; mapped += chunk) {
        hipMemGenericAllocationHandle_t h;
        e = hipMemCreate(&h, chunk, &prop, 0);
        if (e != hipSuccess) break;
        e = hipMemMap((char*)va + mapped, chunk, 0, h, 0);
        if (early_release || e != hipSuccess) (void)hipMemRelease(h); else handles.push_back(h);
        if (e != hipSuccess) break;
    }
    if (e == hipSuccess) {
        hipMemAccessDesc ad = {};
        ad.location.type = hipMemLocationTypeDevice; ad.location.id = ctx->device; ad.flags = hipMemAccessFlagsProtReadWrite;
        e = hipMemSetAccess(va, total, &ad, 1);
    }
    if (e != hipSuccess) {
        if (mapped) (void)hipMemUnmap(va, mapped);
        for (auto h : handles) (void)hipMemRelease(h);
        (void)hipMemAddressFree(va, total);
        return e;
    }
    if (exp_env("SMC_VMM_CLEAR")) { (void)hipMemset(va, 0, total); (void)hipDeviceSynchronize(); }
    {
        std::lock_guard<std::mutex> g(ctx->vmm_mu);
        ctx->vmm.push_back({va, total, handles});
    }
    *out = va;
    return hipSuccess;
}
int smc_mem_alloc(smc_ctx* ctx, int64_t bytes, void** out) {
    if (!ctx || !out || bytes < 0) return fail(SMC_E_ARG, "smc_mem_alloc: bad argument");
    HIPCHK(hipSetDevice(ctx->device));
    size_t chunk_mb = 0;
    { const char* v = exp_env("SMC_VMM_CHUNK_MB"); if (v && *v) chunk_mb = (size_t)std::max(0, atoi(v)); }
    if (chunk_mb > 0 && (size_t)bytes >= ((size_t)SMC_VMM_MIN_MB << 20)) {
        if (vmm_alloc(ctx, (size_t)bytes, chunk_mb << 20, out) == hipSuccess) return SMC_OK;
        (void)hipGetLastError();
    }
    HIPCHK(hipMalloc(out, (size_t)(bytes > 0 ? bytes : 1)));
    return SMC_OK;
}
void smc_mem_free(smc_ctx* ctx, void* p) {
    if (!ctx || !p) return;
    (void)hipSetDevice(ctx->device);
    size_t total = 0;
    std::vector<hipMemGenericAllocationHandle_t> handles;
    {
        std::lock_guard<std::mutex> g(ctx->vmm_mu);
        for (size_t i = 0; i < ctx->vmm.size(); ++i)
            if (ctx->vmm[i].va == p) { total = ctx->vmm[i].total; handles.swap(ctx->vmm[i].handles); ctx->vmm.erase(ctx->vmm.begin() + (long)i); break; }
    }
    if (total) {
        (void)hipDeviceSynchronize();
        (void)hipMemUnmap(p, total);
        for (auto h : handles) (void)hipMemRelease(h);
        (void)hipMemAddressFree(p, total);
        return;
    }
    (void)hipFree(p);
}
// ... 113 lines not shown
```

### smcounter_amd/csrc/k_bp_emit2.inc

```
#define BP2_G 16
#ifndef BP2_ABL
#define BP2_ABL 0
#endif
#ifndef BP2_STORE_AUX
#define BP2_STORE_AUX 0
#endif
#define BP2_LIN_SPAN 4096u
#define BP2_SIMPLE 1u
#define BP2_MQOK 2u
#define BP2_R2 4u
#define BP2_FARA 8u
#define BP2_FARP 16u
#define BP2_SLOW 0x8000u
#define BP2_UNFLAG 0x00800000u
#define BP2_LIN_LANES 16
#define BP2_C_NONE 0x01u
#define BP2_C_GAP 0x08u
#define BP2_C_INS 0x0Au
#define BP2_C_DELS 0x0Cu
#define BP_ST_NOPAIR 16u
struct BpRow { int32_t pos; uint32_t len; uint32_t wbase; uint32_t hi; int32_t cA, cP; uint32_t bc, pair; };
static_assert(sizeof(BpRow) == 32, "two 16-byte loads per row");

__device__ __forceinline__ uint32_t bp2_aux(const uint32_t* __restrict__ rec, const uint32_t* __restrict__ cig) {
    const uint32_t nc = rec[4] & 0xFFFFu;
    if (nc < 1u || nc > 3u) return 0u;
    const uint32_t* c = cig + rec[2];
    const uint32_t w0 = c[0], w1 = nc > 1u ? c[1] : 0x5u, w2 = nc > 2u ? c[2] : 0x5u;
    auto is_m = [](uint32_t x) { const uint32_t o = x & 15u; return o == 0u || o == 7u || o == 8u; };
    auto is_c = [](uint32_t x) { const uint32_t o = x & 15u; return o == 4u || o == 5u; };
    if (is_m(w0) && is_c(w1) && is_c(w2) && nc <= 2u) return 0x80000000u;
    if (is_c(w0) && is_m(w1) && is_c(w2)) return 0x80000000u | ((w0 & 15u) == 4u ? min(w0 >> 4, 0xFFFFu) : 0u);
    return 0u;
}
__device__ __forceinline__ uint32_t bp2_lin_need(uint32_t aux, int pos, int end) {
    if (aux >> 31) return 0u;
    const uint32_t span = end > pos ? (uint32_t)(end - pos) : 0u;
    return (span == 0u || span > BP2_LIN_SPAN) ? 0u : ((span + 31u) & ~15u) + 64u;
}
__global__ __launch_bounds__(256) void k_bp_zero_words(uint32_t* __restrict__ p, uint32_t n) {
    for (uint32_t i = blockIdx.x * 256u + threadIdx.x; i < n; i += gridDim.x * 256u) p[i] = 0u;
}

struct BpRes { int qpos, indel; bool isdel; };
template <typename CIGP>
__device__ __forceinline__ BpRes bp2_resolve(CIGP c, int n_cig, int kpos, int p, int l_seq) {
    BpRes r; r.qpos = -1; r.indel = 0; r.isdel = false;
    int x = kpos, y = 0;
    for (int ci = 0; ci < n_cig; ++ci) {
        const uint32_t wv = c[ci];
        const int op = (int)(wv & 15u), len = (int)(wv >> 4);
        const bool ref_op = op == 0 || op == 7 || op == 8, gap_op = op == 2 || op == 3;
        if (ref_op || gap_op) {
            const int d = p - x;
            if ((uint32_t)d < (uint32_t)len) {
                r.qpos = ref_op ? y + d : y;
                r.isdel = gap_op;
                if (d == len - 1 && ci + 1 < n_cig) {
                    const uint32_t nw = c[ci + 1];
                    r.indel = (nw & 15u) == 1u ? (int)(nw >> 4) : (nw & 15u) == 2u ? -(int)(nw >> 4) : 0;
                }
            }
            x += len;
            if (ref_op) y += len;
            if (x > p) break;
        } else if (op == 1 || op == 4) y += len;
    }
    if (r.isdel && r.indel != 0 && r.qpos >= l_seq) r.indel = 0;
    return r;
}

__global__ __launch_bounds__(256) void k_bp_rows_write(BpArgs A, uint32_t n_aln, uint32_t* __restrict__ cursors , uint32_t* __restrict__ glist, uint32_t glist_stride,
                                                       BpRow* __restrict__ rows, uint32_t lin_cap, int raw, uint2* __restrict__ k8,
                                                       uint32_t* __restrict__ zero, uint32_t zero_words, uint32_t* __restrict__ counters) {
    __shared__ uint32_t ws[4], wc[4], base_cnt;
    __shared__ unsigned long long base_pool;
    const int tid = threadIdx.x, lane = tid & 63, wid = tid >> 6;
    for (uint32_t i = blockIdx.x * 256u + threadIdx.x; i < zero_words; i += gridDim.x * 256u) zero[i] = 0u;
    if (blockIdx.x == 0 && threadIdx.x < 2) counters[threadIdx.x] = 0u;
    const uint32_t a = blockIdx.x * 256u + (uint32_t)tid;
    const bool valid = a < n_aln;
    uint32_t nd = 0;
    if (valid) {
        const uint32_t* rec0 = (const uint32_t*)(A.aln + a);
        nd = bp2_lin_need(bp2_aux(rec0, A.cig), (int)rec0[0], (int)rec0[1]);
    }
    uint32_t inc = nd;
    for (int o = 1; o < 64; o <<= 1) { const uint32_t u = (uint32_t)__shfl_up((int)inc, o); if (lane >= o) inc += u; }
    const unsigned long long gm = __builtin_amdgcn_ballot_w64(nd != 0u);
    if (lane == 63) { ws[wid] = inc; wc[wid] = (uint32_t)__popcll(gm); }
    __syncthreads();
    if (tid == 0) {
        const uint32_t ts = ws[0] + ws[1] + ws[2] + ws[3], tc = wc[0] + wc[1] + wc[2] + wc[3];
        uint32_t* const cur = cursors + 32u * (blockIdx.x % BP_NCUR);
        base_pool = ts ? atomicAdd((unsigned long long*)cur, (unsigned long long)ts) : 0ull;
        base_cnt = tc ? atomicAdd(&cur[2], tc) : 0u;
    }
    __syncthreads();
    const uint32_t region = lin_cap / BP_NCUR;
    unsigned long long pre = base_pool;
    uint32_t gpre = (blockIdx.x % BP_NCUR) * glist_stride + base_cnt;
    for (int w = 0; w < wid; ++w) { pre += ws[w]; gpre += wc[w]; }
    if (nd != 0u) glist[gpre + bp_lanes_below(gm)] = a;
    const unsigned long long loc64 = 16ull + pre + inc - nd;
    const unsigned long long off64 = (unsigned long long)(blockIdx.x % BP_NCUR) * region + loc64;
    bool lin = false;
    uint32_t off = 0;
    int kpos = 0, kend = 0;
    uint32_t kcig = 0, kseq = 0, k4 = 0, k5 = 0, k6 = 0;
    if (valid) {
        const uint32_t* rec = (const uint32_t*)(A.aln + a);
        kpos = (int)rec[0]; kend = (int)rec[1]; kcig = rec[2]; kseq = rec[3]; k4 = rec[4]; k5 = rec[5]; k6 = rec[6];
        const uint32_t aux = bp2_aux(rec, A.cig);
        const bool simple = aux >> 31;
        const bool unfl = !(((k4 >> 16) & 0xFFu) & (SMC_DA_R1 | SMC_DA_R2));
        lin = !simple && nd != 0u && !raw && !unfl && loc64 + nd <= (unsigned long long)region && (k4 & 0xFFFFu) <= 64u;
        off = (uint32_t)off64;
        off += ((uint32_t)(kpos - A.start0) - off) & 63u;
        const uint32_t oflag = (k4 >> 16) & 0xFFu, mapq = k4 >> 24;
        const bool r2 = (oflag & SMC_DA_R2) != 0, rev = (oflag & SMC_DA_REV) != 0, mmok = (oflag & SMC_DA_MMOK) != 0;
        const bool mq_ok = (int)mapq >= A.min_mq && mmok;
        const bool farA = r2 != rev, farP = r2 && rev;
        const uint32_t cb0 = A.w16 ? 3u + (rev ? 2u : 0u) : 6u + (rev ? 8u : 0u), cinc = A.w16 ? 16u + (r2 ? 5u : 3u) + (rev ? 6u : 0u) : cb0 + (r2 ? 4u : 2u);
        BpRow R;
        R.pos = kpos; R.len = kend > kpos ? (uint32_t)(kend - kpos) : 0u;
        R.hi = ((r2 ? 1u : 0u) | (rev ? 2u : 0u) | (mmok ? 4u : 0u)) << 16 | mapq << 24 | (simple ? BP2_SIMPLE : 0u) | (mq_ok ? BP2_MQOK : 0u) |
               (r2 ? BP2_R2 : 0u) | (farA ? BP2_FARA : 0u) | (farP ? BP2_FARP : 0u) | cb0 << 5 | cinc << 10 | (((!simple && !lin) || unfl) ? BP2_SLOW : 0u) |
               (unfl ? BP2_UNFLAG : 0u);
        const int base = (int)(aux & 0xFFFFu) - (int)(k5 & 0xFFFFu) - kpos, fbase = (int)(k5 >> 16) + 1 - base;
        R.cA = farA ? fbase : base;
        R.cP = r2 ? (farP ? fbase : base) : (1 << 29);
        R.wbase = simple ? kseq + (aux & 0xFFFFu) - (uint32_t)kpos : off - (uint32_t)kpos;
        R.bc = rec[7]; R.pair = rec[8];
        k8[a] = make_uint2(R.bc, R.pair);
        uint4* o = (uint4*)(rows + a);
        o[0] = make_uint4((uint32_t)R.pos, R.len, R.wbase, R.hi);
        o[1] = make_uint4((uint32_t)R.cA, (uint32_t)R.cP, R.bc, R.pair);
    }
}

__global__ __launch_bounds__(256) void k_bp_lin(BpArgs A, const uint32_t* __restrict__ glist, uint32_t glist_stride, const uint32_t* __restrict__ cursors,
                                                BpRow* __restrict__ rows, uint8_t* __restrict__ lin_bq) {
    const int lane = threadIdx.x & (BP2_LIN_LANES - 1);
    constexpr uint32_t TPW = 256u / BP2_LIN_LANES;
    const uint32_t part = blockIdx.x % BP_NCUR, wg_per = max(1u, gridDim.x / BP_NCUR), ng = cursors[32u * part + 2u];
    const bool gap_ok = A.min_bq >= 0 && A.min_bq <= 126;
    if (blockIdx.x / BP_NCUR >= wg_per) return;
    for (uint32_t w = (blockIdx.x / BP_NCUR) * TPW + threadIdx.x / BP2_LIN_LANES; w < ng; w += wg_per * TPW) {
        const uint32_t a = glist[part * glist_stride + w];
        const BpRow R = rows[a];
        if ((R.hi & BP2_SLOW) || (R.hi & BP2_SIMPLE)) continue;
        const uint32_t* rec = (const uint32_t*)(A.aln + a);
        const int kpos = (int)rec[0], kend = (int)rec[1];
        const uint32_t kcig = rec[2], kseq = rec[3], k4 = rec[4], k5 = rec[5];
        const int n_cig = (int)(k4 & 0xFFFFu), l_seq = (int)(rec[6] & 0xFFFFu), left_sp = (int)(k5 & 0xFFFFu), qalen = (int)(k5 >> 16);
        const uint32_t off = R.wbase + (uint32_t)kpos;
        const int span = kend - kpos;
        const bool r2 = (R.hi & BP2_R2) != 0, farA = (R.hi & BP2_FARA) != 0, farP = (R.hi & BP2_FARP) != 0;
        const uint32_t* const cg = A.cig + kcig;
        uint8_t* const out = lin_bq + 2ull * off;
        const uint8_t* const src = A.bq + 2ull * kseq;
        int a_max = kpos - 1, a_min = kend, p_max = kpos - 1, p_min = kend;
        int x = 0, y = 0;
        for (int ci = 0; ci < n_cig; ++ci) {
            const uint32_t wv = cg[ci], nx = ci + 1 < n_cig ? cg[ci + 1] : 0u;
            const int op = (int)(wv & 15u), len = (int)(wv >> 4);
            const bool indel_next = ((nx & 15u) == 1u || (nx & 15u) == 2u) && (nx >> 4) != 0u;
            if (op == 0 || op == 7 || op == 8) {
                const int nd = min(len, span - x);
                for (int d0 = lane; d0 < nd; d0 += 4 * BP2_LIN_LANES) {
                    uint32_t sq[4];
#pragma unroll
                    for (int u = 0; u < 4; ++u) { const int d = d0 + u * BP2_LIN_LANES; sq[u] = (d < nd && y + d < l_seq) ? *(const uint16_t*)(src + 2 * (y + d)) : 0u; }
#pragma unroll
                    for (int u = 0; u < 4; ++u) {
                        const int d = d0 + u * BP2_LIN_LANES;
                        if (d >= nd) break;
                        uint32_t site = sq[u] & 0xFFu, bq = sq[u] >> 8;
                        if (d == len - 1 && indel_next) { site = y + d < l_seq ? ((nx & 15u) == 1u ? BP2_C_INS : BP2_C_DELS) : BP2_C_NONE; bq = min(bq, 127u); }
                        else if (y + d >= l_seq) { site = BP2_C_NONE; bq = 0u; }
                        *(uint16_t*)(out + 2 * (x + d)) = (uint16_t)(site | bq << 8);
                    }
                }
                {
                    const int lastd = len - 1 - (indel_next ? 1 : 0), px = kpos + x;
                    auto upto = [&](int lim) { return min(lastd, lim + left_sp - y); };
                    auto from = [&](int lim) { return max(0, qalen - lim + left_sp - y); };
                    if (!farA) { const int d = upto(20); if (d >= 0) a_max = max(a_max, px + d); }
                    else { const int d = from(20); if (d <= lastd) a_min = min(a_min, px + d); }
                    if (r2) {
                        if (!farP) { const int d = upto(A.primer_dist); if (d >= 0) p_max = max(p_max, px + d); }
                        else { const int d = from(A.primer_dist); if (d <= lastd) p_min = min(p_min, px + d); }
                    }
                }
                x += len; y += len;
            } else if (op == 2 || op == 3) {
                for (int d = lane; d < len && x + d < span; d += BP2_LIN_LANES) {
                    const bool odd = d == len - 1 && indel_next && y < l_seq;
                    const uint32_t site = (odd || !gap_ok) ? BP2_C_NONE : BP2_C_GAP;
                    *(uint16_t*)(out + 2 * (x + d)) = (uint16_t)(site | (site == BP2_C_GAP ? (uint32_t)A.min_bq << 8 : 0u));
                }
                x += len;
            } else if (op == 1 || op == 4) y += len;
        }
        for (int d = max(x, 0) + lane; d < span; d += BP2_LIN_LANES) *(uint16_t*)(out + 2 * d) = (uint16_t)BP2_C_NONE;
        if (lane == 0) {
            int32_t* o = (int32_t*)(rows + a);
            o[4] = farA ? a_min + 21 : 20 - a_max;
            o[5] = !r2 ? (1 << 29) : farP ? p_min + A.primer_dist + 1 : A.primer_dist - p_max;
        }
    }
}

__device__ __forceinline__ uint32_t bp2_seg_scan(uint32_t M, unsigned long long S, uint32_t carry, uint32_t& pre) {
    uint32_t x = M;
    const unsigned long long A1 = S, A2 = A1 | (A1 << 1), A4 = A2 | (A2 << 2), A8 = A4 | (A4 << 4);
    auto take = [&](unsigned long long keep, uint32_t t) { x |= __builtin_amdgcn_inverse_ballot_w64(keep) ? t : 0u; };
    take(~A1, (uint32_t)__builtin_amdgcn_update_dpp(0, (int)x, 0x111, 0xF, 0xF, true));
    take(~A2, (uint32_t)__builtin_amdgcn_update_dpp(0, (int)x, 0x112, 0xF, 0xF, true));
    take(~A4, (uint32_t)__builtin_amdgcn_update_dpp(0, (int)x, 0x114, 0xF, 0xF, true));
    take(~A8, (uint32_t)__builtin_amdgcn_update_dpp(0, (int)x, 0x118, 0xF, 0xF, true));
    unsigned long long P = S;
    P |= (P << 1) & ~0x0001000100010001ull; P |= (P << 2) & ~0x0003000300030003ull;
    P |= (P << 4) & ~0x000F000F000F000Full; P |= (P << 8) & ~0x00FF00FF00FF00FFull;
    take(~P & 0xFFFF0000FFFF0000ull, (uint32_t)__builtin_amdgcn_update_dpp(0, (int)x, 0x142, 0xA, 0xF, false));
    const unsigned long long Q = P | (((P >> 47) & 1ull) ? 0xFFFF000000000000ull : 0ull);
    take(~Q & 0xFFFFFFFF00000000ull, (uint32_t)__builtin_amdgcn_update_dpp(0, (int)x, 0x143, 0xC, 0xF, false));
    const unsigned long long first = S ? ((S & (0ull - S)) - 1ull) : ~0ull;
    const uint32_t cin = __builtin_amdgcn_inverse_ballot_w64(first) ? carry : 0u;
    const uint32_t prev = (uint32_t)__builtin_amdgcn_update_dpp(0, (int)x, 0x138, 0xF, 0xF, true);
    pre = (__builtin_amdgcn_inverse_ballot_w64(~S) ? prev : 0u) | cin;
    return x | cin;
}
__device__ __forceinline__ void bp2_writelane(uint32_t& v, uint32_t s, int k) {
    asm volatile("v_writelane_b32 %0, %1, %2" : "+v"(v) : "s"(s), "n"(k));
}
__device__ __forceinline__ uint32_t bp2_wave_or(uint32_t v) {
    for (int o = 32; o; o >>= 1) v |= (uint32_t)__shfl_xor((int)v, o);
    return v;
}
__device__ __forceinline__ uint32_t bp2_cover(int d0, uint32_t len, int ng) {
    const int lo = min(max(-d0, 0), BP2_G), hi = min(max((int)len - d0, 0), ng);
    return hi > lo ? ((1u << hi) - 1u) & ~((1u << lo) - 1u) : 0u;
}

typedef uint32_t bp2_u4 __attribute__((ext_vector_type(4)));
__device__ __forceinline__ void bp2_gload4(bp2_u4& d, const void* p) { asm volatile("global_load_dwordx4 %0, %1, off" : "=v"(d) : "v"(p) : "memory"); }
__device__ __forceinline__ void bp2_gload1(uint32_t& d, const void* p) { asm volatile("global_load_dword %0, %1, off" : "=v"(d) : "v"(p) : "memory"); }
__device__ __forceinline__ unsigned long long bp2_cover64(int d0, uint32_t len, int nt) {
    const int lo = min(max(-d0, 0), 64), hi = min(max((int)len - d0, 0), nt);
    if (hi <= lo) return 0ull;
    return (hi >= 64 ? ~0ull : ((1ull << hi) - 1ull)) & ~((1ull << lo) - 1ull);
}
__device__ __forceinline__ unsigned long long bp2_seg_scan64(unsigned long long M, unsigned long long S, unsigned long long carry, unsigned long long& pre) {
    uint32_t x0 = (uint32_t)M, x1 = (uint32_t)(M >> 32);
    const unsigned long long A1 = S, A2 = A1 | (A1 << 1), A4 = A2 | (A2 << 2), A8 = A4 | (A4 << 4);
    unsigned long long P = S;
    P |= (P << 1) & ~0x0001000100010001ull; P |= (P << 2) & ~0x0003000300030003ull;
    P |= (P << 4) & ~0x000F000F000F000Full; P |= (P << 8) & ~0x00FF00FF00FF00FFull;
    const unsigned long long Q = P | (((P >> 47) & 1ull) ? 0xFFFF000000000000ull : 0ull);
#define BP2_TAKE(keep, ctrl, rm, bc)                                                                             \
    {                                                                                                            \
        const bool kp = __builtin_amdgcn_inverse_ballot_w64(keep);                                               \
        const uint32_t t0 = (uint32_t)__builtin_amdgcn_update_dpp(0, (int)x0, ctrl, rm, 0xF, bc);               \
        const uint32_t t1 = (uint32_t)__builtin_amdgcn_update_dpp(0, (int)x1, ctrl, rm, 0xF, bc);               \
        x0 |= kp ? t0 : 0u; x1 |= kp ? t1 : 0u;                                                                  \
    }
    BP2_TAKE(~A1, 0x111, 0xF, true) BP2_TAKE(~A2, 0x112, 0xF, true) BP2_TAKE(~A4, 0x114, 0xF, true) BP2_TAKE(~A8, 0x118, 0xF, true)
    BP2_TAKE(~P & 0xFFFF0000FFFF0000ull, 0x142, 0xA, false) BP2_TAKE(~Q & 0xFFFFFFFF00000000ull, 0x143, 0xC, false)
#undef BP2_TAKE
    const unsigned long long first = S ? ((S & (0ull - S)) - 1ull) : ~0ull;
    const bool fl = __builtin_amdgcn_inverse_ballot_w64(first), ns = __builtin_amdgcn_inverse_ballot_w64(~S);
    const uint32_t c0 = fl ? (uint32_t)carry : 0u, c1 = fl ? (uint32_t)(carry >> 32) : 0u;
    const uint32_t p0 = (uint32_t)__builtin_amdgcn_update_dpp(0, (int)x0, 0x138, 0xF, 0xF, true), p1 = (uint32_t)__builtin_amdgcn_update_dpp(0, (int)x1, 0x138, 0xF, 0xF, true);
    pre = (unsigned long long)((ns ? p0 : 0u) | c0) | (unsigned long long)((ns ? p1 : 0u) | c1) << 32;
    return (unsigned long long)(x0 | c0) | (unsigned long long)(x1 | c1) << 32;
}
__device__ __forceinline__ unsigned long long bp2_rl64(unsigned long long v, int l) {
    return (unsigned long long)(uint32_t)__builtin_amdgcn_readlane((int)(uint32_t)v, l) |
           (unsigned long long)(uint32_t)__builtin_amdgcn_readlane((int)(uint32_t)(v >> 32), l) << 32;
}

template <bool RAW , bool W16 >
__global__ __launch_bounds__(64) void k_bp_emit2(BpArgs A, const BpRow* __restrict__ rows, const uint8_t* __restrict__ lin_bq) {
    __shared__ uint32_t xq[BP_XQ * BP_XW];
    __shared__ uint32_t stage[(BP2_ABL & 0x8000) ? 33 * 68 : 1];
    const int lane = threadIdx.x;
// ... 403 lines not shown
```

### smcounter_amd/csrc/k_build_planes.inc

```
#define BP_TILE 64
#define BP_SEG_TILES_DEEP 8
#define BP_RS_TILE 1024
#define BP_RS_MAXBLK 4096
#ifndef BP_SORT_WAVES
#define BP_SORT_WAVES 16
#endif
#define BP_SORT_LDS_MAX 6144
#ifndef BP_SORT_WAVES_SMALL
#define BP_SORT_WAVES_SMALL 8
#endif
#define BP_SORT_REG (BP_SORT_LDS_MAX / (64 * BP_SORT_WAVES_SMALL))
#define BP_SORT_REG_BIG (BP_LSORT_MAX / (64 * BP_SORT_WAVES))
#define BP_LSORT_MAX 16384
#define BP_XQ 64
#define BP_XREP 256
#define BP_NCUR 64
#define BP_XW 8
#define BP_ST_DEPTH 1u
#define BP_ST_XLIST 2u
#define BP_ST_BQ 4u
#define BP_ST_ALLELES 8u
#define BP_ST_NARROW 32u

struct BpSeg {
    uint32_t w0, w1;
    uint32_t off;
    uint32_t part_base, ppt;
    uint32_t blk_base, n_blk;
    uint32_t n_tiles;
    uint32_t cpart_base, cppt;
};
#define BP_SUB 64

struct BpArgs {
    const smc_dev_aln* aln; const uint32_t* cig; const uint8_t* bq;
    const smc_dev_locus* loc; const uint8_t* refseq;
    int32_t start0, n_loci, n_seg, part;
    int32_t seg_tiles;
    int32_t min_bq, min_mq, primer_dist, ds;
    uint32_t fp;
    uint32_t xcd_rot;
    uint32_t slot_base, umi_base;
    uint32_t *words;
    uint32_t w16;
    uint32_t *meta, *umi, *frag, *dist, *umi_start, *u_gid, *u_finc;
    smc_locus* loci;
    const BpSeg* seg;
    const uint32_t* sorted;
    uint32_t* cnt;
    uint32_t* cntp;
    uint32_t* pstate;
    uint32_t *xraw, xraw_cap, *xraw_n;
    uint32_t *xcnt, *tcnt, *tcur, *gidx;
    uint32_t *gidx2;
    uint32_t *xlist, xcap, *xcount, *status;
};

__device__ __forceinline__ void bp_patch_allele(const BpArgs& A, uint32_t sp, uint32_t id) {
    if (!A.words) return;
    if (A.w16) {
        if (id > 15u) { atomicOr(A.status, BP_ST_NARROW); return; }
        uint8_t* b = (uint8_t*)A.words + 2ull * sp;
        *b = (uint8_t)((*b & 0xF0u) | id);
    } else ((uint8_t*)A.words)[4ull * sp] = (uint8_t)id;
}
__device__ __forceinline__ uint32_t bp_lanes_below(unsigned long long m) {
    return (uint32_t)__builtin_amdgcn_mbcnt_hi((uint32_t)(m >> 32), __builtin_amdgcn_mbcnt_lo((uint32_t)m, 0u));
}
__device__ __forceinline__ void bp_match(uint32_t dgt, bool valid, int nbits, uint32_t& rank, uint32_t& np) {
    const unsigned long long v = __builtin_amdgcn_ballot_w64(valid);
    uint32_t lo = (uint32_t)v, hi = (uint32_t)(v >> 32);
#pragma unroll
    for (int bit = 0; bit < 8; ++bit) {
        if (bit < nbits) {
            const uint32_t x = (uint32_t)(((int)(dgt << (31 - bit))) >> 31);
            const unsigned long long m = __builtin_amdgcn_ballot_w64(x != 0u);
            lo &= ~((uint32_t)m ^ x); hi &= ~((uint32_t)(m >> 32) ^ x);
        }
    }
    rank = __builtin_amdgcn_mbcnt_hi(hi, __builtin_amdgcn_mbcnt_lo(lo, 0u));
    np = (uint32_t)__popc(lo) + (uint32_t)__popc(hi);
}
template <int BY >
__device__ __forceinline__ int bp_seg_of(const BpSeg* __restrict__ seg, int n_seg, uint32_t x) {
    int lo = 0, hi = n_seg - 1;
    while (lo < hi) {
        const int mid = (lo + hi + 1) >> 1;
        const uint32_t b = BY == 1 ? seg[mid].part_base : BY == 2 ? seg[mid].cpart_base : seg[mid].blk_base;
        if (b <= x) lo = mid; else hi = mid - 1;
    }
    return lo;
}
__device__ __forceinline__ unsigned long long bp_key_hash(const smc_dev_aln& a, const uint8_t* __restrict__ bq, int qpos, int indel) {
    unsigned long long h = 1469598103934665603ull;
    auto mix = [&](uint32_t b) { h ^= (unsigned long long)(b & 0xffu); h *= 1099511628211ull; };
    const uint8_t* s = bq + 2ull * a.seq_off;
    mix(indel > 0 ? 'I' : indel < 0 ? 'D' : 'L');
    mix(s[2 * qpos]);
    if (indel > 0) { for (int k = qpos + 1; k < (int)a.l_seq && k < qpos + 1 + indel; ++k) mix(s[2 * k]); }
    else if (indel < 0) { const uint32_t l = (uint32_t)(-indel); mix(l); mix(l >> 8); mix(l >> 16); mix(l >> 24); }
    return h;
}
__device__ __forceinline__ int bp_fixed_allele(uint32_t site) {
    return site == 'A' ? 0 : site == 'T' ? 1 : site == 'G' ? 2 : site == 'C' ? 3 : site == 'N' ? 4 : -1;
}

__host__ __device__ static inline uint32_t bp_seg_blocks(uint32_t cnt, uint32_t max_blk) {
    if (cnt <= BP_LSORT_MAX) return 0u;
    const uint32_t t = (cnt + BP_RS_TILE - 1) / BP_RS_TILE;
    return t < max_blk ? t : max_blk;
}
__global__ __launch_bounds__(1024) void k_bp_segtab(const smc_dev_locus* __restrict__ loc, int n_loci, int n_seg, int seg_loci, uint32_t part, uint32_t max_blk,
                                                    BpSeg* __restrict__ seg) {
    __shared__ uint32_t ws[4][16];
    __shared__ uint32_t carry[4];
    const int tid = threadIdx.x, lane = tid & 63, wid = tid >> 6;
    if (tid < 4) carry[tid] = 0u;
    __syncthreads();
    for (int base = 0; base < n_seg; base += 1024) {
        const int s = base + tid;
        BpSeg S{};
        uint32_t v[4] = {0u, 0u, 0u, 0u};
        if (s < n_seg) {
            const int l0 = s * seg_loci, l1 = min(n_loci, l0 + seg_loci) - 1;
            S.w0 = loc[l0].w0;
            const uint32_t e = loc[l1].w1;
            S.w1 = e > S.w0 ? e : S.w0;
            const uint32_t cnt = S.w1 - S.w0;
            S.n_tiles = (uint32_t)((l1 - l0) / BP_TILE + 1);
            S.ppt = (cnt + BP_SUB - 1) / BP_SUB;
            S.cppt = (cnt + part - 1) / part;
            S.n_blk = bp_seg_blocks(cnt, max_blk);
            v[0] = cnt; v[1] = S.ppt * S.n_tiles; v[2] = S.n_blk; v[3] = S.cppt * S.n_tiles;
        }
        uint32_t ex[4];
#pragma unroll
        for (int c = 0; c < 4; ++c) {
            uint32_t inc = v[c];
            for (int o = 1; o < 64; o <<= 1) { const uint32_t u = (uint32_t)__shfl_up((int)inc, o); if (lane >= o) inc += u; }
            if (lane == 63) ws[c][wid] = inc;
            ex[c] = inc - v[c];
        }
        __syncthreads();
#pragma unroll
        for (int c = 0; c < 4; ++c) {
            uint32_t pre = carry[c];
            for (int w = 0; w < wid; ++w) pre += ws[c][w];
            ex[c] += pre;
        }
        if (s < n_seg) { S.off = ex[0]; S.part_base = ex[1]; S.blk_base = ex[2]; S.cpart_base = ex[3]; seg[s] = S; }
        __syncthreads();
        if (tid < 4) { uint32_t t = 0; for (int w = 0; w < 16; ++w) t += ws[tid][w]; carry[tid] += t; }
        __syncthreads();
    }
}

__global__ __launch_bounds__(1024) void k_bp_scan(uint32_t* __restrict__ d, uint32_t n, const uint32_t* __restrict__ n_dev) {
    __shared__ uint32_t ws[16];
    const int tid = threadIdx.x, lane = tid & 63, wid = tid >> 6;
    if (n_dev) n = min(*n_dev, n) + 1u;
    uint32_t carry = 0;
    constexpr int PER = 16;
    for (uint32_t base = 0; base < n; base += 1024u * PER) {
        const uint32_t i = base + (uint32_t)PER * (uint32_t)tid;
        uint32_t v[PER];
        if (i + PER <= n && (((uintptr_t)(d + i)) & 15u) == 0u) {
#pragma unroll
            for (int k = 0; k < PER; k += 4) { const uint4 q = *(const uint4*)(d + i + k); v[k] = q.x; v[k + 1] = q.y; v[k + 2] = q.z; v[k + 3] = q.w; }
        } else {
#pragma unroll
            for (int k = 0; k < PER; ++k) v[k] = i + k < n ? d[i + k] : 0u;
        }
        uint32_t t = 0;
#pragma unroll
        for (int k = 0; k < PER; ++k) t += v[k];
        uint32_t inc = t;
        for (int o = 1; o < 64; o <<= 1) { const uint32_t u = (uint32_t)__shfl_up((int)inc, o); if (lane >= o) inc += u; }
        if (lane == 63) ws[wid] = inc;
        __syncthreads();
        uint32_t pre = carry, tot = 0;
        for (int w = 0; w < 16; ++w) { const uint32_t x = ws[w]; if (w < wid) pre += x; tot += x; }
        uint32_t run = pre + inc - t;
#pragma unroll
        for (int k = 0; k < PER; ++k) { if (i + k < n) d[i + k] = run; run += v[k]; }
        carry += tot;
        __syncthreads();
    }
}

struct BpBlk { uint32_t e0, e1, hidx, hstride, w0, off, h0; int seg; };
__device__ __forceinline__ BpBlk bp_blk(const BpSeg* __restrict__ seg, int n_seg, uint32_t b) {
    const int s = bp_seg_of<0>(seg, n_seg, b);
    const BpSeg S = seg[s];
    const uint32_t bl = b - S.blk_base, cnt = S.w1 - S.w0, steps = (cnt + BP_RS_TILE - 1) / BP_RS_TILE;
    const uint32_t t0 = (uint32_t)((unsigned long long)bl * steps / S.n_blk), t1 = (uint32_t)((unsigned long long)(bl + 1) * steps / S.n_blk);
    BpBlk B;
    B.e0 = S.off + t0 * BP_RS_TILE;
    const uint32_t e1 = S.off + t1 * BP_RS_TILE, end = S.off + cnt;
    B.e1 = e1 < end ? e1 : end;
    B.hidx = S.blk_base * 256u + bl; B.hstride = S.n_blk;
    B.w0 = S.w0; B.off = S.off; B.h0 = S.blk_base * 256u; B.seg = s;
    return B;
}
template <bool FIRST >
__global__ __launch_bounds__(64) void k_bp_hist(const BpSeg* __restrict__ seg, int n_seg, const uint2* __restrict__ k8, int pair_bits,
                                                unsigned long long* __restrict__ keys, uint32_t* __restrict__ vals, int shift,
                                                uint32_t* __restrict__ hist) {
    __shared__ uint32_t lh[256];
    const int lane = threadIdx.x;
    const BpBlk B = bp_blk(seg, n_seg, blockIdx.x);
#pragma unroll
    for (int k = 0; k < 4; ++k) lh[lane + 64 * k] = 0u;
    __builtin_amdgcn_wave_barrier();
    for (uint32_t e = B.e0 + (uint32_t)lane; e < B.e1; e += 64u) {
        unsigned long long key;
        if (FIRST) {
            const uint32_t a = B.w0 + (e - B.off);
            const uint2 kv = k8[a];
            key = ((unsigned long long)kv.x << pair_bits) | (unsigned long long)kv.y;
            keys[e] = key; vals[e] = a;
        } else key = keys[e];
        atomicAdd(&lh[(uint32_t)(key >> shift) & 255u], 1u);
    }
    __builtin_amdgcn_wave_barrier();
#pragma unroll
    for (int k = 0; k < 4; ++k) { const uint32_t dgt = (uint32_t)lane + 64u * k; hist[B.hidx + dgt * B.hstride] = lh[dgt]; }
}
__global__ __launch_bounds__(64) void k_bp_rowscan(const BpSeg* __restrict__ seg, uint32_t* __restrict__ hist, uint32_t* __restrict__ dtot) {
    const int lane = threadIdx.x;
    const uint32_t s = blockIdx.x >> 8, dgt = blockIdx.x & 255u;
    const BpSeg S = seg[s];
    if (!S.n_blk) { if (lane == 0) dtot[blockIdx.x] = 0u; return; }
    uint32_t* row = hist + (size_t)S.blk_base * 256u + (size_t)dgt * S.n_blk;
    uint32_t carry = 0;
    for (uint32_t b0 = 0; b0 < S.n_blk; b0 += 256u) {
        const uint32_t i = b0 + 4u * (uint32_t)lane;
        uint32_t v[4];
#pragma unroll
        for (int k = 0; k < 4; ++k) v[k] = i + k < S.n_blk ? row[i + k] : 0u;
        const uint32_t t = v[0] + v[1] + v[2] + v[3];
        uint32_t inc = t;
        for (int o = 1; o < 64; o <<= 1) { const uint32_t u = (uint32_t)__shfl_up((int)inc, o); if (lane >= o) inc += u; }
        uint32_t run = carry + inc - t;
#pragma unroll
        for (int k = 0; k < 4; ++k) { if (i + k < S.n_blk) row[i + k] = run; run += v[k]; }
        carry += (uint32_t)__builtin_amdgcn_readlane((int)inc, 63);
    }
    if (lane == 0) dtot[blockIdx.x] = carry;
}
__global__ __launch_bounds__(64) void k_bp_scatter(const BpSeg* __restrict__ seg, int n_seg, const unsigned long long* __restrict__ kin,
                                                   const uint32_t* __restrict__ vin, unsigned long long* __restrict__ kout,
                                                   uint32_t* __restrict__ vout, int shift, const uint32_t* __restrict__ hist,
                                                   const uint32_t* __restrict__ dtot) {
    __shared__ uint32_t offs[256];
    const int lane = threadIdx.x;
    const BpBlk B = bp_blk(seg, n_seg, blockIdx.x);
    {
        uint32_t v[4], t = 0;
#pragma unroll
        for (int k = 0; k < 4; ++k) { v[k] = dtot[(uint32_t)B.seg * 256u + 4u * (uint32_t)lane + (uint32_t)k]; t += v[k]; }
        uint32_t inc = t;
        for (int o = 1; o < 64; o <<= 1) { const uint32_t u = (uint32_t)__shfl_up((int)inc, o); if (lane >= o) inc += u; }
        uint32_t run = B.off + inc - t;
#pragma unroll
        for (int k = 0; k < 4; ++k) { offs[4 * lane + k] = run; run += v[k]; }
    }
    __builtin_amdgcn_wave_barrier();
#pragma unroll
    for (int k = 0; k < 4; ++k) { const uint32_t dgt = (uint32_t)lane + 64u * k; offs[dgt] += hist[B.hidx + dgt * B.hstride]; }
    __builtin_amdgcn_wave_barrier();
    for (uint32_t e0 = B.e0; e0 < B.e1; e0 += 64u) {
        const uint32_t e = e0 + (uint32_t)lane;
        const bool valid = e < B.e1;
        unsigned long long key = 0; uint32_t val = 0;
        if (valid) { key = kin[e]; val = vin[e]; }
        const uint32_t dgt = (uint32_t)(key >> shift) & 255u;
        uint32_t rank, n;
        bp_match(dgt, valid, 8, rank, n);
        const uint32_t base = valid ? offs[dgt] : 0u;
        __builtin_amdgcn_wave_barrier();
        if (valid && rank == 0u) offs[dgt] = base + n;
        __builtin_amdgcn_wave_barrier();
        if (valid) { kout[base + rank] = key; vout[base + rank] = val; }
    }
}

struct BpReg16 {
    uint32_t a[4], b[4], c[4], d[4];
    __device__ __forceinline__ uint32_t& at(int i) { return i < 4 ? a[i] : i < 8 ? b[i - 4] : i < 12 ? c[i - 8] : d[i - 12]; }
};
template <int REG , int WAVES , bool BIG>
__global__ __launch_bounds__(64 * WAVES) void k_bp_sort_seg(const BpSeg* __restrict__ seg, const uint2* __restrict__ k8 , int pair_bits, int passes,
                                                      unsigned long long* k0, unsigned long long* k1, uint32_t* v0, uint32_t* v1, uint32_t only_above, uint32_t only_upto) {
    constexpr int LDS_MAX = 64 * WAVES * REG;
    if (!BIG && (seg[blockIdx.x].w1 - seg[blockIdx.x].w0) > only_upto) return;
    __shared__ uint32_t whist[WAVES][256];
    __shared__ uint32_t dtot[256], dbase[256];
    const BpSeg S = seg[blockIdx.x];
    const uint32_t n = S.w1 - S.w0;
    if (n == 0u || n > BP_LSORT_MAX || (BIG ? n <= only_above : false)) return;
    const int tid = threadIdx.x, lane = tid & 63, wid = tid >> 6;
    const uint32_t chunk = ((n + (uint32_t)WAVES - 1u) / (uint32_t)WAVES + 63u) & ~63u;
    const uint32_t e0 = min(n, (uint32_t)wid * chunk), e1 = min(n, e0 + chunk);
    unsigned long long* kb[2] = {k0 + S.off, k1 + S.off};
    uint32_t* vb[2] = {v0 + S.off, v1 + S.off};
    __shared__ uint32_t rng[4];
    if (tid == 0) { rng[0] = 0xFFFFFFFFu; rng[1] = 0u; rng[2] = 0xFFFFFFFFu; rng[3] = 0u; }
    __syncthreads();
    {
        uint32_t b_lo = 0xFFFFFFFFu, b_hi = 0u, p_lo = 0xFFFFFFFFu, p_hi = 0u;
        for (uint32_t e = e0 + (uint32_t)lane; e < e1; e += 64u) {
            const uint2 kv = k8[S.w0 + e];
            const uint32_t b = kv.x, q = kv.y;
            b_lo = min(b_lo, b); b_hi = max(b_hi, b); p_lo = min(p_lo, q); p_hi = max(p_hi, q);
        }
        for (int o = 32; o; o >>= 1) {
            b_lo = min(b_lo, (uint32_t)__shfl_xor((int)b_lo, o)); b_hi = max(b_hi, (uint32_t)__shfl_xor((int)b_hi, o));
            p_lo = min(p_lo, (uint32_t)__shfl_xor((int)p_lo, o)); p_hi = max(p_hi, (uint32_t)__shfl_xor((int)p_hi, o));
        }
        if (lane == 0 && e0 < e1) { atomicMin(&rng[0], b_lo); atomicMax(&rng[1], b_hi); atomicMin(&rng[2], p_lo); atomicMax(&rng[3], p_hi); }
    }
    __syncthreads();
    const uint32_t bc_min = rng[0], pair_min = rng[2];
    const int pb = 32 - __builtin_clz((rng[3] - pair_min) | 1u), bb = 32 - __builtin_clz((rng[1] - bc_min) | 1u);
    int my_passes = (pb + bb + 7) / 8;
    if (pb + bb > 8 * passes) my_passes = passes;
    (void)pair_bits;
    if (n <= (uint32_t)LDS_MAX && pb + bb <= 32 && chunk <= 64u * REG) {
        __shared__ uint32_t lk[LDS_MAX];
        __shared__ uint16_t lv[LDS_MAX];
        static_assert(LDS_MAX <= 65536, "lv holds window indices in 16 bits");
        BpReg16 key, val;
#pragma unroll
        for (int it = 0; it < REG; ++it) {
            const uint32_t e = e0 + 64u * (uint32_t)it + (uint32_t)lane;
            key.at(it) = 0u; val.at(it) = 0u;
            if (e < e1) {
                val.at(it) = e;
                const uint2 kv = k8[S.w0 + e];
                key.at(it) = (kv.x - bc_min) << pb | (kv.y - pair_min);
            }
        }
        typedef __attribute__((address_space(1))) uint32_t glb_u32;
        glb_u32* const out = (glb_u32*)vb[passes & 1];
        const int dbits = __builtin_amdgcn_readfirstlane(max(1, (pb + bb + my_passes - 1) / max(1, my_passes)));
        const uint32_t dmask = (1u << dbits) - 1u;
        for (int ps = 0; ps < my_passes; ++ps) {
            const int shift = dbits * ps;
            const bool last = ps == my_passes - 1;
#pragma unroll
            for (int k = 0; k < 4; ++k) whist[wid][lane + 64 * k] = 0u;
            __builtin_amdgcn_wave_barrier();
#pragma unroll
            for (int it = 0; it < REG; ++it)
                if (e0 + 64u * (uint32_t)it + (uint32_t)lane < e1) atomicAdd(&whist[wid][(key.at(it) >> shift) & dmask], 1u);
            __syncthreads();
            if (tid < 256) {
                uint32_t run = 0;
#pragma unroll
                for (int w = 0; w < WAVES; ++w) { const uint32_t v = whist[w][tid]; whist[w][tid] = run; run += v; }
                dtot[tid] = run;
            }
            __syncthreads();
            if (wid == 0) {
                uint32_t v[4], t = 0;
#pragma unroll
                for (int k = 0; k < 4; ++k) { v[k] = dtot[4 * lane + k]; t += v[k]; }
                uint32_t inc = t;
                for (int o = 1; o < 64; o <<= 1) { const uint32_t u = (uint32_t)__shfl_up((int)inc, o); if (lane >= o) inc += u; }
                uint32_t run = inc - t;
#pragma unroll
                for (int k = 0; k < 4; ++k) { dbase[4 * lane + k] = run; run += v[k]; }
            }
            __syncthreads();
#pragma unroll
            for (int it = 0; it < REG; ++it) {
                if (e0 + 64u * (uint32_t)it >= e1) break;
                const bool valid = e0 + 64u * (uint32_t)it + (uint32_t)lane < e1;
                const uint32_t dgt = valid ? (key.at(it) >> shift) & dmask : 0u;
                uint32_t rank, np;
                bp_match(dgt, valid, dbits, rank, np);
                const uint32_t wo = valid ? whist[wid][dgt] : 0u;
                __builtin_amdgcn_wave_barrier();
                if (valid && rank == 0u) whist[wid][dgt] = wo + np;
                __builtin_amdgcn_wave_barrier();
                if (valid) {
                    const uint32_t d = dbase[dgt] + wo + rank;
                    if (last) out[d] = S.w0 + val.at(it);
                    else { lk[d] = key.at(it); lv[d] = (uint16_t)val.at(it); }
                }
            }
            if (last) break;
            __syncthreads();
#pragma unroll
            for (int it = 0; it < REG; ++it) {
                const uint32_t e = e0 + 64u * (uint32_t)it + (uint32_t)lane;
                if (e < e1) { key.at(it) = lk[e]; val.at(it) = lv[e]; }
            }
            __syncthreads();
        }
        return;
    }
    my_passes += (passes - my_passes) & 1;
    for (int ps = 0; ps < my_passes; ++ps) {
        const int shift = 8 * ps;
        const unsigned long long* kin = kb[ps & 1];
        const uint32_t* vin = vb[ps & 1];
        unsigned long long* kout = kb[(ps & 1) ^ 1];
        uint32_t* vout = vb[(ps & 1) ^ 1];
        auto fetch = [&](uint32_t e, unsigned long long& key, uint32_t& val) {
            if (ps == 0) {
                val = S.w0 + e;
                const uint2 kv = k8[val];
                key = ((unsigned long long)(kv.x - bc_min) << pb) | (unsigned long long)(kv.y - pair_min);
            } else { key = kin[e]; val = vin[e]; }
        };
#pragma unroll
        for (int k = 0; k < 4; ++k) whist[wid][lane + 64 * k] = 0u;
        __builtin_amdgcn_wave_barrier();
        for (uint32_t e = e0 + (uint32_t)lane; e < e1; e += 64u) {
            unsigned long long key; uint32_t val;
            fetch(e, key, val);
            atomicAdd(&whist[wid][(uint32_t)(key >> shift) & 255u], 1u);
        }
        __syncthreads();
        if (tid < 256) {
            uint32_t run = 0;
#pragma unroll
            for (int w = 0; w < WAVES; ++w) { const uint32_t v = whist[w][tid]; whist[w][tid] = run; run += v; }
            dtot[tid] = run;
        }
        __syncthreads();
        if (wid == 0) {
            uint32_t v[4], t = 0;
#pragma unroll
            for (int k = 0; k < 4; ++k) { v[k] = dtot[4 * lane + k]; t += v[k]; }
            uint32_t inc = t;
            for (int o = 1; o < 64; o <<= 1) { const uint32_t u = (uint32_t)__shfl_up((int)inc, o); if (lane >= o) inc += u; }
            uint32_t run = inc - t;
#pragma unroll
            for (int k = 0; k < 4; ++k) { dbase[4 * lane + k] = run; run += v[k]; }
        }
        __syncthreads();
        for (uint32_t eb = e0; eb < e1; eb += 64u) {
            const uint32_t e = eb + (uint32_t)lane;
            const bool valid = e < e1;
            unsigned long long key = 0; uint32_t val = 0;
            if (valid) fetch(e, key, val);
            const uint32_t dgt = (uint32_t)(key >> shift) & 255u;
            uint32_t rank, np;
            bp_match(dgt, valid, 8, rank, np);
            const uint32_t wo = valid ? whist[wid][dgt] : 0u;
            __builtin_amdgcn_wave_barrier();
            if (valid && rank == 0u) whist[wid][dgt] = wo + np;
            __builtin_amdgcn_wave_barrier();
            if (valid) { const uint32_t d = dbase[dgt] + wo + rank; kout[d] = key; vout[d] = val; }
        }
        __syncthreads();
    }
}

struct BpWave {
    int tile, l, p, p_first, p_last;
    bool active;
    uint32_t a_lo, a_hi, seg_off, j0, j1, jb, sub0, cpart, csub;
};
template <bool COUNT >
__device__ __forceinline__ BpWave bp_wave(const BpArgs& A, int lane, uint32_t w) {
    BpWave W;
    const int s = bp_seg_of<COUNT ? 2 : 1>(A.seg, A.n_seg, w);
    const BpSeg SG = A.seg[s];
    const uint32_t rr = w - (COUNT ? SG.cpart_base : SG.part_base), ppt = COUNT ? SG.cppt : SG.ppt, part = COUNT ? (uint32_t)A.part : (uint32_t)BP_SUB;
    const uint32_t tis = rr / ppt, q = rr - tis * ppt;
    W.tile = s * A.seg_tiles + (int)tis;
    const int l_first = W.tile * BP_TILE;
    const int l_last = min(A.n_loci, l_first + BP_TILE) - 1;
    W.l = l_first + lane;
    W.active = W.l <= l_last;
    W.p = A.start0 + W.l; W.p_first = A.start0 + l_first; W.p_last = A.start0 + l_last;
    W.a_lo = A.loc[l_first].w0; W.a_hi = A.loc[l_last].w1;
    W.seg_off = SG.off;
    const uint32_t seg_end = SG.off + (SG.w1 - SG.w0);
    W.j0 = SG.off + q * part;
    W.j1 = min(seg_end, W.j0 + part);
    W.sub0 = SG.part_base + tis * SG.ppt + q * (part / (uint32_t)BP_SUB);
    {
        const uint32_t per = (uint32_t)A.part / (uint32_t)BP_SUB;
        W.cpart = SG.cpart_base + tis * SG.cppt + q / per; W.csub = q % per;
    }
    W.jb = W.j0;
    if (COUNT && W.j0 > SG.off && W.j0 < W.j1) {
        const uint32_t bc0 = A.aln[A.sorted[W.j0]].bc_gid;
        while (W.jb > SG.off) {
            const uint32_t base = W.jb - SG.off >= 64u ? W.jb - 64u : SG.off;
            const uint32_t j = base + (uint32_t)lane;
            const bool in = j < W.jb;
            const uint32_t b = in ? A.aln[A.sorted[j]].bc_gid : bc0;
            const unsigned long long other = __builtin_amdgcn_ballot_w64(in && b != bc0);
            if (other) { W.jb = base + (uint32_t)(63 - __builtin_clzll(other)) + 1u; break; }
            W.jb = base;
        }
    }
    return W;
}
__device__ __forceinline__ uint32_t bp_scan_xor(uint32_t v) {
    v ^= (uint32_t)__builtin_amdgcn_update_dpp(0, (int)v, 0x111, 0xF, 0xF, true);
    v ^= (uint32_t)__builtin_amdgcn_update_dpp(0, (int)v, 0x112, 0xF, 0xF, true);
    v ^= (uint32_t)__builtin_amdgcn_update_dpp(0, (int)v, 0x114, 0xF, 0xF, true);
    v ^= (uint32_t)__builtin_amdgcn_update_dpp(0, (int)v, 0x118, 0xF, 0xF, true);
    v ^= (uint32_t)__builtin_amdgcn_update_dpp(0, (int)v, 0x142, 0xA, 0xF, false);
    v ^= (uint32_t)__builtin_amdgcn_update_dpp(0, (int)v, 0x143, 0xC, 0xF, false);
    return v;
}
#include "bp_masks.h"
#define BP_MASK_LDS (66 + 32 + 32)
struct BpCols { uint32_t C, NF, NB; };
__device__ __forceinline__ BpCols bp_columns(uint32_t* lds, int lane, bool in_b, uint32_t rr, uint32_t nrows, int lo, int hi, uint32_t bc,
                                             uint32_t pair, uint32_t& last_bc, uint32_t& last_pair) {
    uint32_t* const ev = lds;
    uint32_t* const rbc = lds + 66;
    uint32_t* const rpair = rbc + 32;
    ev[lane] = 0u;
    if (lane < 2) ev[64 + lane] = 0u;
    __builtin_amdgcn_wave_barrier();
    if (in_b) { atomicOr(&ev[lo], 1u << rr); atomicOr(&ev[hi], 1u << rr); rbc[rr] = bc; rpair[rr] = pair; }
    __builtin_amdgcn_wave_barrier();
    BpCols R;
    R.C = bp_scan_xor(ev[lane]);
    const uint32_t x = rbc[lane & 31], xp = rbc[(lane - 1) & 31], y = rpair[lane & 31], yp = rpair[(lane - 1) & 31];
    const bool row = lane >= 1 && (uint32_t)lane < nrows;
    const uint32_t SB = (uint32_t)__builtin_amdgcn_ballot_w64(row && x == xp), SP = (uint32_t)__builtin_amdgcn_ballot_w64(row && y == yp);
    R.NB = bp_heads(R.C, SB, last_bc == rbc[0]);
    R.NF = bp_heads(R.C, SP, last_pair == rpair[0]);
    if (R.C) { const int top = 31 - __builtin_clz(R.C); last_bc = rbc[top]; last_pair = rpair[top]; }
    __builtin_amdgcn_wave_barrier();
    return R;
}
struct BpRec { int pos, end; uint32_t bc, pair; bool inwin; };
__device__ __forceinline__ uint32_t bp_batch_index(const BpArgs& A, uint32_t c0, uint32_t c_to, int lane) {
    const uint32_t j = c0 + (uint32_t)lane;
    return j < c_to ? A.sorted[j] : 0xFFFFFFFFu;
}
__device__ __forceinline__ BpRec bp_batch_rec(const BpArgs& A, const BpWave& W, uint32_t a) {
    BpRec R; R.pos = 0x7FFFFFFF; R.end = 0; R.bc = 0; R.pair = 0;
    R.inwin = a != 0xFFFFFFFFu && a >= W.a_lo && a < W.a_hi;
    if (R.inwin) { const uint32_t* rec = (const uint32_t*)(A.aln + a); R.pos = (int)rec[0]; R.end = (int)rec[1]; R.bc = rec[7]; R.pair = rec[8]; }
    return R;
}
template <bool COUNT>
__device__ __forceinline__ void bp_walk_batch(const BpWave& W, int lane, const BpRec& R, uint32_t& last_bc, uint32_t& last_pair, uint32_t& c_r,
                                              uint32_t& c_f, uint32_t& c_u, uint32_t* lds) {
    const bool ov = R.inwin && R.end > W.p_first && R.pos <= W.p_last;
    const unsigned long long todo = __builtin_amdgcn_ballot_w64(ov);
    if (!todo) return;
    const uint32_t r = bp_lanes_below(todo), n = (uint32_t)__popcll(todo);
    const int lo = max(R.pos - W.p_first, 0), hi = min(R.end - W.p_first, 64);
    for (uint32_t b0 = 0; b0 < n; b0 += 32u) {
        const BpCols K = bp_columns(lds, lane, ov && r >= b0 && r < b0 + 32u, r - b0, min(32u, n - b0), lo, hi, R.bc, R.pair, last_bc, last_pair);
        if (COUNT) { c_r += (uint32_t)__popc(K.C); c_f += (uint32_t)__popc(K.NF); c_u += (uint32_t)__popc(K.NB); }
    }
}

__global__ __launch_bounds__(64) void k_bp_count(BpArgs A) {
    __shared__ uint32_t lds[BP_MASK_LDS];
    const int lane = threadIdx.x;
    const BpWave W = bp_wave<true>(A, lane, blockIdx.x);
    uint32_t last_bc = 0xFFFFFFFFu, last_pair = 0xFFFFFFFFu, c_r = 0, c_f = 0, c_u = 0;
    uint32_t s_bc = 0, s_pair = 0;
    {
        const uint32_t c0 = W.j0 + (uint32_t)BP_SUB * (uint32_t)lane;
        if (c0 < W.j1) { const smc_dev_aln* r0 = A.aln + A.sorted[c0]; s_bc = r0->bc_gid; s_pair = r0->pair_gid; }
    }
    const uint32_t n_rep = W.j0 > W.jb ? (W.j0 - W.jb + 63u) / 64u : 0u, n_main = W.j1 > W.j0 ? (W.j1 - W.j0 + (uint32_t)BP_SUB - 1u) / (uint32_t)BP_SUB : 0u;
    const uint32_t n_bat = n_rep + n_main;
    auto bounds = [&](uint32_t k, uint32_t& b0, uint32_t& b1) {
        if (k < n_rep) { b0 = W.jb + 64u * k; b1 = min(W.j0, b0 + 64u); }
        else { b0 = W.j0 + (uint32_t)BP_SUB * (k - n_rep); b1 = min(W.j1, b0 + (uint32_t)BP_SUB); }
    };
    auto index_of = [&](uint32_t k) -> uint32_t {
        if (k >= n_bat) return 0xFFFFFFFFu;
        uint32_t b0, b1; bounds(k, b0, b1);
        return bp_batch_index(A, b0, b1, lane);
    };
    uint32_t a_next = index_of(0);
    BpRec R = bp_batch_rec(A, W, a_next);
    a_next = index_of(1);
    uint32_t sub = W.sub0, t_r = 0, t_f = 0, t_u = 0;
    for (uint32_t k = 0; k < n_bat; ++k) {
        const BpRec Rn = bp_batch_rec(A, W, a_next);
        a_next = index_of(k + 2u);
        if (k < n_rep) { bp_walk_batch<false>(W, lane, R, last_bc, last_pair, c_r, c_f, c_u, lds); R = Rn; continue; }
        const uint32_t i = k - n_rep;
        {
            const uint32_t bc0 = (uint32_t)__builtin_amdgcn_readlane((int)s_bc, (int)(i & 63u)), pair0 = (uint32_t)__builtin_amdgcn_readlane((int)s_pair, (int)(i & 63u));
            const unsigned long long cb = __builtin_amdgcn_ballot_w64(last_bc == bc0), cp = __builtin_amdgcn_ballot_w64(last_pair == pair0);
            if (lane < 4) A.pstate[(size_t)sub * 4u + (uint32_t)lane] = lane == 0 ? (uint32_t)cb : lane == 1 ? (uint32_t)(cb >> 32) : lane == 2 ? (uint32_t)cp : (uint32_t)(cp >> 32);
        }
        c_r = c_f = c_u = 0;
        bp_walk_batch<true>(W, lane, R, last_bc, last_pair, c_r, c_f, c_u, lds);
        A.cntp[(size_t)sub * 64u + (uint32_t)lane] = c_r | c_f << 8 | c_u << 16;
        t_r += c_r; t_f += c_f; t_u += c_u;
        ++sub;
        R = Rn;
    }
    uint32_t* const cw = A.cnt + (size_t)blockIdx.x * 192u;
    cw[lane] = t_r; cw[64 + lane] = t_f; cw[128 + lane] = t_u;
}

#define BP_TL_CH 4096
__global__ __launch_bounds__(256) void k_bp_tile_count(const BpSeg* __restrict__ sseg, int seg_tiles, const BpSeg* __restrict__ wseg, int n_tiles, int nch,
                                                       const uint32_t* __restrict__ sorted, uint32_t* __restrict__ tc) {
    __shared__ uint32_t ws[4];
    const int tid = threadIdx.x, lane = tid & 63, wid = tid >> 6;
    const int tile = blockIdx.x / nch, c = blockIdx.x % nch;
    const BpSeg S = sseg[tile / seg_tiles], W = wseg[tile];
    const uint32_t cnt = S.w1 - S.w0, e0 = (uint32_t)c * BP_TL_CH, e1 = min(cnt, e0 + BP_TL_CH);
    uint32_t m = 0;
    for (uint32_t e = e0 + (uint32_t)tid; e < e1; e += 256u) { const uint32_t a = sorted[S.off + e]; m += (a >= W.w0 && a < W.w1) ? 1u : 0u; }
    for (int o = 32; o; o >>= 1) m += (uint32_t)__shfl_xor((int)m, o);
    if (lane == 0) ws[wid] = m;
    __syncthreads();
    if (tid == 0) tc[blockIdx.x] = ws[0] + ws[1] + ws[2] + ws[3];
}
__global__ __launch_bounds__(256) void k_bp_tile_scatter(const BpSeg* __restrict__ sseg, int seg_tiles, const BpSeg* __restrict__ wseg, int n_tiles, int nch,
                                                         const uint32_t* __restrict__ sorted, const uint32_t* __restrict__ tc, uint32_t* __restrict__ sorted2) {
    __shared__ uint32_t ws[4], wbase;
    const int tid = threadIdx.x, lane = tid & 63, wid = tid >> 6;
    const int tile = blockIdx.x / nch, c = blockIdx.x % nch;
    const BpSeg S = sseg[tile / seg_tiles], W = wseg[tile];
    const uint32_t cnt = S.w1 - S.w0, e0 = (uint32_t)c * BP_TL_CH, e1 = min(cnt, e0 + BP_TL_CH);
    if (e0 >= e1) return;
    uint32_t before = 0;
    for (int k = tid; k < c; k += 256) before += tc[(size_t)tile * nch + k];
    for (int o = 32; o; o >>= 1) before += (uint32_t)__shfl_xor((int)before, o);
    if (lane == 0) ws[wid] = before;
    __syncthreads();
    uint32_t base = W.off + ws[0] + ws[1] + ws[2] + ws[3];
    __syncthreads();
    for (uint32_t r0 = e0; r0 < e1; r0 += 256u) {
        const uint32_t e = r0 + (uint32_t)tid;
        const uint32_t a = e < e1 ? sorted[S.off + e] : 0xFFFFFFFFu;
        const bool hit = e < e1 && a >= W.w0 && a < W.w1;
        const unsigned long long hm = __builtin_amdgcn_ballot_w64(hit);
        if (lane == 0) ws[wid] = (uint32_t)__popcll(hm);
        __syncthreads();
        uint32_t pre = base;
        for (int w = 0; w < wid; ++w) pre += ws[w];
        if (hit) sorted2[pre + bp_lanes_below(hm)] = a;
        base += ws[0] + ws[1] + ws[2] + ws[3];
        __syncthreads();
    }
}

__global__ __launch_bounds__(256) void k_bp_scan_tiles(BpArgs A) {
    __shared__ uint32_t ws[4][3][64];
    const int tid = threadIdx.x, lane = tid & 63, wid = tid >> 6;
    const int tile = blockIdx.x, s = tile / A.seg_tiles;
    const BpSeg SG = A.seg[s];
    const uint32_t P = SG.cppt;
    uint32_t* const base = A.cnt + ((size_t)SG.cpart_base + (size_t)(tile - s * A.seg_tiles) * P) * 192u;
    const uint32_t q0 = P * (uint32_t)wid / 4u, q1 = P * (uint32_t)(wid + 1) / 4u;
    uint32_t sum[3] = {0u, 0u, 0u};
#pragma unroll 4
    for (uint32_t q = q0; q < q1; ++q) {
        const uint32_t* c = base + (size_t)q * 192u;
        sum[0] += c[lane]; sum[1] += c[64 + lane]; sum[2] += c[128 + lane];
    }
// ... 257 lines not shown
```

Measured before the change: 79.77 million.

## Drop dead alignment rows during segment sort and bound partitions by live count

The rows-write kernel now records each alignment's end coordinate, and the per-segment sort filters out rows that end before the segment's first locus. The sort compacts only live rows and writes a per-segment live count. Downstream wave partitioning uses that count instead of the full segment length. This is meant to skip scanning alignments that cannot cover any locus in the tile, at the cost of an extra end-position array, extra filtering logic in the sort, and a new live-count table. The filter is enabled only when there is one tile per segment, unless an experimental environment variable keeps dead rows.

```diff
diff --git a/include/smcounter_hip.h b/include/smcounter_hip.h
--- a/include/smcounter_hip.h
+++ b/include/smcounter_hip.h
@@ -483,6 +483,7 @@
 int smc_build_max_depth(void);
 int smc_build_set_timing(smc_ctx* ctx, int slots);
 int smc_build_kernel_ms(smc_ctx* ctx, float* avg_ms, int32_t* n_samples);
+int smc_build_live_rows(smc_ctx* ctx, uint32_t* live, int32_t cap, int32_t* n_lists);
 int smc_build_planes(smc_ctx* ctx, const smc_params* params, const smc_build_in* in, uint32_t slot_base, uint32_t umi_base,
                      uint32_t* words, uint32_t* meta, uint32_t* umi, uint32_t* frag, uint32_t* dist, uint32_t* umi_start,
                      uint32_t* u_gid, uint32_t* u_finc, smc_locus* loci, uint32_t* xlist, uint32_t xcap, uint32_t* counters, void* stream);
diff --git a/smcounter_amd/_lib.py b/smcounter_amd/_lib.py
--- a/smcounter_amd/_lib.py
+++ b/smcounter_amd/_lib.py
@@ -14,7 +14,7 @@
            "smc_read_groups_counts_frac", "smc_read_groups_masks_grid", "smc_read_groups_kept_grid", "smc_lod_table", "smc_fisher_tables", "smc_lfact_values", "smc_allele_carriers", "smc_af_rep_masks", "smc_af_rep_counts", "smc_af_depth_masks", "smc_af_depth_counts", "smc_spike_alleles", "smc_spike_indels", "smc_spike_alleles_reps", "smc_spike_rep_counts", "smc_spike_depth_counts", "smc_spike_phase_counts", "smc_spike_indels_reps", "smc_spike_indel_touch", "smc_spike_indel_counts", "smc_spike_indel_phase_counts", "smc_spike_read_bits", "smc_spike_rpb_counts", "smc_spike_indel_read_bits", "smc_spike_indel_rpb_counts", "smc_spike_phase_rpb_counts", "smc_read_groups_counts_frac_seeds", "smc_spike_grid_counts", "smc_scan_detect", "smc_scan_detect_keys", "smc_scan_filter", "smc_plan_destroy", "smc_plan_info",
            "smc_plan_run", "smc_plan_run_words", "smc_plan_run_words16", "smc_pack_words", "smc_plan_set_timing", "smc_plan_kernel_ms", "smc_call_batch_host", "smc_event_create", "smc_event_record",
            "smc_event_elapsed_ms", "smc_event_destroy", "smc_class_table", "smc_wire_row_size", "smc_pack_rows", "smc_unpack_rows",
-           "smc_build_planes", "smc_build_planes_w16", "smc_build_listed", "smc_build_max_depth", "smc_build_set_timing", "smc_build_kernel_ms", "smc_mem_alloc", "smc_mem_alloc_best", "smc_mem_write_probe", "smc_mem_free", "smc_mem_h2d", "smc_mem_d2h",
+           "smc_build_planes", "smc_build_planes_w16", "smc_build_listed", "smc_build_max_depth", "smc_build_set_timing", "smc_build_kernel_ms", "smc_build_live_rows", "smc_mem_alloc", "smc_mem_alloc_best", "smc_mem_write_probe", "smc_mem_free", "smc_mem_h2d", "smc_mem_d2h",
            "smc_mem_alloc_host", "smc_mem_free_host", "smc_pool_trim",
            "smc_device_sync")
 
@@ -141,6 +141,7 @@
     L.smc_build_max_depth.restype = ctypes.c_int
     L.smc_build_set_timing.argtypes = [vp, ctypes.c_int]
     L.smc_build_kernel_ms.argtypes = [vp, ctypes.POINTER(ctypes.c_float), ctypes.POINTER(ctypes.c_int32)]
+    L.smc_build_live_rows.argtypes = [vp, vp, ctypes.c_int32, ctypes.POINTER(ctypes.c_int32)]
     L.smc_build_planes.argtypes = [vp, ctypes.POINTER(abi.SmcParams), ctypes.POINTER(abi.SmcBuildIn), ctypes.c_uint32,
                                    ctypes.c_uint32, vp, vp, vp, vp, vp, vp, vp, vp, vp, vp, ctypes.c_uint32, vp, vp]
     L.smc_build_planes_w16.argtypes = [vp, ctypes.POINTER(abi.SmcParams), ctypes.POINTER(abi.SmcBuildIn), ctypes.c_uint32,
diff --git a/smcounter_amd/csrc/bp_masks.h b/smcounter_amd/csrc/bp_masks.h
--- a/smcounter_amd/csrc/bp_masks.h
+++ b/smcounter_amd/csrc/bp_masks.h
@@ -14,3 +14,9 @@
     if (carried) H &= ~G0;
     return H;
 }
+BP_HD bool bp_row_dead(int end , int p_first ) { return end <= p_first; }
+BP_HD void bp_part_rows(uint32_t off, uint32_t n_live, uint32_t q, uint32_t part, uint32_t& j0, uint32_t& j1) {
+    const uint32_t end = off + n_live;
+    j0 = off + q * part;
+    j1 = end < j0 + part ? end : j0 + part;
+}
diff --git a/smcounter_amd/csrc/host_abi.inc b/smcounter_amd/csrc/host_abi.inc
--- a/smcounter_amd/csrc/host_abi.inc
+++ b/smcounter_amd/csrc/host_abi.inc
@@ -41,6 +41,8 @@
     int seg_next = 0;
     std::vector<hipEvent_t> bp_ev0, bp_ev1;
     int64_t bp_timed = 0;
+    size_t bp_nlive_off = 0;
+    int32_t bp_nlive_n = 0;
     std::vector<std::pair<size_t, void*>> plan_pool;
     struct PendingFree { hipEvent_t ev; std::vector<std::pair<size_t, void*>> blocks; };
     std::vector<PendingFree> plan_pending;
@@ -2376,8 +2378,8 @@
     const uint32_t xraw_cap = (uint32_t)std::min<uint64_t>(1u << 28, reads / 32 + 65536);
     size_t off = 0;
     auto carve = [&](size_t bytes) { const size_t o = off; off += (bytes + 255) & ~(size_t)255; return o; };
-    const size_t o_seg = carve(sizeof(BpSeg) * (size_t)n_seg);
-    const size_t o_wseg = carve(tile_lists ? sizeof(BpSeg) * (size_t)n_tiles : 0), o_sorted2 = carve(tile_lists ? 4 * (size_t)ntot_w : 0),
+    const size_t o_seg = carve((sizeof(BpSeg) + 4) * (size_t)n_seg);
+    const size_t o_wseg = carve(tile_lists ? (sizeof(BpSeg) + 4) * (size_t)n_tiles : 0), o_sorted2 = carve(tile_lists ? 4 * (size_t)ntot_w : 0),
                  o_tc = carve(tile_lists ? 4 * (size_t)n_tiles * (size_t)nch : 0);
     const size_t o_k0 = carve(8 * (size_t)ntot), o_k1 = carve(8 * (size_t)ntot), o_v0 = carve(4 * (size_t)ntot), o_v1 = carve(4 * (size_t)ntot);
     const size_t o_hist = carve(4 * 256 * (size_t)total_blk), o_dtot = carve(4 * 256 * (size_t)n_seg);
@@ -2388,6 +2390,7 @@
     const size_t o_bsum = carve(128 * BP_NCUR + 256), o_lin = carve(2 * lin_cap + 256);
     const uint32_t glist_stride = 256u * ((n_rblk + BP_NCUR - 1) / BP_NCUR) + 64u;
     const size_t o_glist = carve(4 * (size_t)glist_stride * BP_NCUR), o_k8 = carve(8 * (size_t)std::max<int64_t>(1, n_aln));
+    const size_t o_kend = carve(4 * (size_t)std::max<int64_t>(1, n_aln));
     const size_t o_zero = off;
     const size_t o_xcnt = carve(4 * (size_t)n_loci), o_tcnt = carve(4 * ((size_t)n_tiles + 1)), o_tcur = carve(4 * (size_t)n_tiles), o_xn = carve(4);
     const size_t o_zend = off;
@@ -2411,7 +2414,9 @@
     A.words = words; A.w16 = w16 ? 1u : 0u; A.meta = meta; A.umi = umi; A.frag = frag; A.dist = dist; A.umi_start = umi_start; A.u_gid = u_gid; A.u_finc = u_finc;
     A.loci = loci;
     BpSeg* d_seg = (BpSeg*)(sc + o_seg);
-    A.seg = d_seg;
+    uint32_t* d_nlive = (uint32_t*)(d_seg + n_seg);
+    A.seg = d_seg; A.n_live = d_nlive;
+    const bool live_rows = tiles_per_seg == 1 && !exp_env("SMC_BP_KEEP_DEAD_ROWS");
     A.cnt = (uint32_t*)(sc + o_cnt); A.cntp = (uint32_t*)(sc + o_cntp); A.pstate = (uint32_t*)(sc + o_pstate);
     A.xraw = (uint32_t*)(sc + o_xraw); A.xraw_cap = xraw_cap; A.xraw_n = (uint32_t*)(sc + o_xn);
     A.xcnt = (uint32_t*)(sc + o_xcnt); A.tcnt = (uint32_t*)(sc + o_tcnt); A.tcur = (uint32_t*)(sc + o_tcur); A.gidx = (uint32_t*)(sc + o_gidx); A.gidx2 = (uint32_t*)(sc + o_gidx2);
@@ -2422,15 +2427,16 @@
         ctx->seg_next = (ctx->seg_next + 1) % 4;
         if (SG.used) HIPCHK(hipEventSynchronize(SG.ev));
         const size_t n_stage = (size_t)n_seg + (tile_lists ? (size_t)n_tiles : 0);
-        if (SG.cap < sizeof(BpSeg) * n_stage) {
+        if (SG.cap < (sizeof(BpSeg) + 4) * n_stage) {
             if (SG.host) (void)hipHostFree(SG.host);
             SG.host = nullptr; SG.cap = 0;
-            const size_t want = std::max<size_t>(4096, sizeof(BpSeg) * n_stage * 2);
+            const size_t want = std::max<size_t>(4096, (sizeof(BpSeg) + 4) * n_stage * 2);
             HIPCHK(hipHostMalloc(&SG.host, want, hipHostMallocDefault));
             SG.cap = want;
         }
         if (!SG.ev) HIPCHK(hipEventCreateWithFlags(&SG.ev, hipEventDisableTiming));
         BpSeg* hs = (BpSeg*)SG.host;
+        uint32_t* hn = (uint32_t*)(hs + n_seg);
         uint32_t off_run = 0, part_run = 0, blk_run = 0, cpart_run = 0;
         for (int sgi = 0; sgi < n_seg; ++sgi) {
             BpSeg S{};
@@ -2444,11 +2450,12 @@
             S.n_blk = bp_seg_blocks(cnt, max_blk);
             S.off = off_run; S.part_base = part_run; S.blk_base = blk_run; S.cpart_base = cpart_run;
             off_run += cnt; part_run += S.ppt * S.n_tiles; blk_run += S.n_blk; cpart_run += S.cppt * S.n_tiles;
-            hs[(size_t)sgi] = S;
+            hs[(size_t)sgi] = S; hn[(size_t)sgi] = cnt;
         }
-        HIPCHK(hipMemcpyAsync(d_seg, hs, sizeof(BpSeg) * (size_t)n_seg, hipMemcpyHostToDevice, st));
+        HIPCHK(hipMemcpyAsync(d_seg, hs, (sizeof(BpSeg) + 4) * (size_t)n_seg, hipMemcpyHostToDevice, st));
         if (tile_lists) {
-            BpSeg* hw = hs + n_seg;
+            BpSeg* hw = (BpSeg*)(hn + n_seg);
+            uint32_t* hwn = (uint32_t*)(hw + n_tiles);
             uint32_t woff = 0, wpart = 0, wcpart = 0;
             for (int t = 0; t < n_tiles; ++t) {
                 BpSeg S{};
@@ -2458,24 +2465,26 @@
                 S.n_tiles = 1u; S.ppt = (cnt + BP_SUB - 1) / BP_SUB; S.cppt = (cnt + part - 1) / part; S.n_blk = 0u;
                 S.off = woff; S.part_base = wpart; S.blk_base = 0u; S.cpart_base = wcpart;
                 woff += cnt; wpart += S.ppt; wcpart += S.cppt;
-                hw[(size_t)t] = S;
+                hw[(size_t)t] = S; hwn[(size_t)t] = cnt;
             }
-            HIPCHK(hipMemcpyAsync(d_wseg, hw, sizeof(BpSeg) * (size_t)n_tiles, hipMemcpyHostToDevice, st));
+            HIPCHK(hipMemcpyAsync(d_wseg, hw, (sizeof(BpSeg) + 4) * (size_t)n_tiles, hipMemcpyHostToDevice, st));
         }
         HIPCHK(hipEventRecord(SG.ev, st));
         SG.used = true;
     } else
-        hipLaunchKernelGGL(k_bp_segtab, dim3(1), dim3(1024), 0, st, in->loc, n_loci, n_seg, seg_loci, part, max_blk, d_seg);
+        hipLaunchKernelGGL(k_bp_segtab, dim3(1), dim3(1024), 0, st, in->loc, n_loci, n_seg, seg_loci, part, max_blk, d_seg, d_nlive);
     HIPCHK(hipGetLastError());
     const bool raw = meta || umi || frag || dist;
     BpRow* d_rows = (BpRow*)(sc + o_rows);
     uint8_t* d_lin = (uint8_t*)(sc + o_lin);
     uint2* d_k8 = (uint2*)(sc + o_k8);
+    int32_t* d_kend = (int32_t*)(sc + o_kend);
+    uint32_t* const sort_nlive = live_rows ? d_nlive : nullptr;
     uint32_t* d_bsum = (uint32_t*)(sc + o_bsum);
     uint32_t* d_glist = (uint32_t*)(sc + o_glist);
     if (total_parts) {
         hipLaunchKernelGGL(k_bp_zero_words, dim3(8), dim3(256), 0, st, d_bsum, 32u * BP_NCUR);
-        hipLaunchKernelGGL(k_bp_rows_write, dim3(n_rblk), dim3(256), 0, st, A, (uint32_t)n_aln, d_bsum, d_glist, glist_stride, d_rows, (uint32_t)lin_cap, raw ? 1 : 0, d_k8,
+        hipLaunchKernelGGL(k_bp_rows_write, dim3(n_rblk), dim3(256), 0, st, A, (uint32_t)n_aln, d_bsum, d_glist, glist_stride, d_rows, (uint32_t)lin_cap, raw ? 1 : 0, d_k8, d_kend,
                            (uint32_t*)(sc + o_zero), (uint32_t)((o_zend - o_zero) / 4), counters);
     }
     unsigned long long* kb[2] = {(unsigned long long*)(sc + o_k0), (unsigned long long*)(sc + o_k1)};
@@ -2493,10 +2502,10 @@
         for (int s = 0; s < n_seg; ++s) any_le |= seg_cnt[(size_t)s] > 0 && seg_cnt[(size_t)s] <= BP_SORT_LDS_MAX;
         if (any_le || !big)
             hipLaunchKernelGGL((k_bp_sort_seg<BP_SORT_REG, BP_SORT_WAVES_SMALL, false>), dim3((unsigned)n_seg), dim3(64 * BP_SORT_WAVES_SMALL), 0, st, d_seg, d_k8, pair_bits, passes, kb[0], kb[1], vb[0], vb[1],
-                               0u, big ? (uint32_t)BP_SORT_LDS_MAX : (uint32_t)BP_LSORT_MAX);
+                               0u, big ? (uint32_t)BP_SORT_LDS_MAX : (uint32_t)BP_LSORT_MAX, d_kend, in->start0, sort_nlive);
         if (big)
             hipLaunchKernelGGL((k_bp_sort_seg<BP_SORT_REG_BIG, BP_SORT_WAVES, true>), dim3((unsigned)n_seg), dim3(64 * BP_SORT_WAVES), 0, st, d_seg, d_k8, pair_bits, passes, kb[0], kb[1], vb[0], vb[1],
-                               (uint32_t)BP_SORT_LDS_MAX, (uint32_t)BP_LSORT_MAX);
+                               (uint32_t)BP_SORT_LDS_MAX, (uint32_t)BP_LSORT_MAX, d_kend, in->start0, sort_nlive);
     }
     if (total_blk) {
         for (int ps = 0; ps < passes; ++ps) {
@@ -2517,7 +2526,7 @@
         const unsigned tgrid = (unsigned)((size_t)n_tiles * (size_t)nch);
         hipLaunchKernelGGL(k_bp_tile_count, dim3(tgrid), dim3(256), 0, st, d_seg, tiles_per_seg, d_wseg, n_tiles, nch, A.sorted, d_tc);
         hipLaunchKernelGGL(k_bp_tile_scatter, dim3(tgrid), dim3(256), 0, st, d_seg, tiles_per_seg, d_wseg, n_tiles, nch, A.sorted, d_tc, d_sorted2);
-        A.sorted = d_sorted2; A.seg = d_wseg; A.n_seg = n_tiles; A.seg_tiles = 1;
+        A.sorted = d_sorted2; A.seg = d_wseg; A.n_live = (const uint32_t*)(d_wseg + n_tiles); A.n_seg = n_tiles; A.seg_tiles = 1;
     }
     if (total_parts) {
         int64_t lin_grid = 2048;
@@ -2543,6 +2552,7 @@
         hipLaunchKernelGGL(k_bp_xfix, dim3((unsigned)n_tiles), dim3(64 * BP_XF_WAVES), 0, st, A);
     }
     HIPCHK(hipGetLastError());
+    ctx->bp_nlive_off = (size_t)((const char*)A.n_live - sc); ctx->bp_nlive_n = A.n_seg;
     if (!ctx->bp_done_ev) HIPCHK(hipEventCreateWithFlags(&ctx->bp_done_ev, hipEventDisableTiming));
     HIPCHK(hipEventRecord(ctx->bp_done_ev, st));
     return SMC_OK;
@@ -2624,6 +2634,17 @@
     return SMC_OK;
 }
 
+int smc_build_live_rows(smc_ctx* ctx, uint32_t* live, int32_t cap, int32_t* n_lists) {
+    if (!ctx || !n_lists || cap < 0 || (cap > 0 && !live)) return fail(SMC_E_ARG, "smc_build_live_rows: bad argument");
+    if (!ctx->bp_scratch || !ctx->bp_done_ev || ctx->bp_nlive_n <= 0) return fail(SMC_E_ARG, "smc_build_live_rows: no build on this context yet");
+    HIPCHK(hipSetDevice(ctx->device));
+    HIPCHK(hipEventSynchronize(ctx->bp_done_ev));
+    *n_lists = ctx->bp_nlive_n;
+    const int32_t n = std::min(cap, ctx->bp_nlive_n);
+    if (n > 0) HIPCHK(hipMemcpy(live, (const char*)ctx->bp_scratch + ctx->bp_nlive_off, 4 * (size_t)n, hipMemcpyDeviceToHost));
+    return SMC_OK;
+}
+
 int smc_build_set_timing(smc_ctx* ctx, int slots) {
     if (!ctx || slots < 0) return fail(SMC_E_ARG, "smc_build_set_timing: bad argument");
     HIPCHK(hipSetDevice(ctx->device));
diff --git a/smcounter_amd/csrc/k_bp_emit2.inc b/smcounter_amd/csrc/k_bp_emit2.inc
--- a/smcounter_amd/csrc/k_bp_emit2.inc
+++ b/smcounter_amd/csrc/k_bp_emit2.inc
@@ -72,7 +72,7 @@
 
 __global__ __launch_bounds__(256) void k_bp_rows_write(BpArgs A, uint32_t n_aln, uint32_t* __restrict__ cursors , uint32_t* __restrict__ glist, uint32_t glist_stride,
                                                        BpRow* __restrict__ rows, uint32_t lin_cap, int raw, uint2* __restrict__ k8,
-                                                       uint32_t* __restrict__ zero, uint32_t zero_words, uint32_t* __restrict__ counters) {
+                                                       int32_t* __restrict__ k_end , uint32_t* __restrict__ zero, uint32_t zero_words, uint32_t* __restrict__ counters) {
     __shared__ uint32_t ws[4], wc[4], base_cnt;
     __shared__ unsigned long long base_pool;
     const int tid = threadIdx.x, lane = tid & 63, wid = tid >> 6;
@@ -133,6 +133,7 @@
         R.wbase = simple ? kseq + (aux & 0xFFFFu) - (uint32_t)kpos : off - (uint32_t)kpos;
         R.bc = rec[7]; R.pair = rec[8];
         k8[a] = make_uint2(R.bc, R.pair);
+        k_end[a] = kend;
         uint4* o = (uint4*)(rows + a);
         o[0] = make_uint4((uint32_t)R.pos, R.len, R.wbase, R.hi);
         o[1] = make_uint4((uint32_t)R.cA, (uint32_t)R.cP, R.bc, R.pair);
diff --git a/smcounter_amd/csrc/k_build_planes.inc b/smcounter_amd/csrc/k_build_planes.inc
--- a/smcounter_amd/csrc/k_build_planes.inc
+++ b/smcounter_amd/csrc/k_build_planes.inc
@@ -46,6 +46,7 @@
     uint32_t *meta, *umi, *frag, *dist, *umi_start, *u_gid, *u_finc;
     smc_locus* loci;
     const BpSeg* seg;
+    const uint32_t* n_live;
     const uint32_t* sorted;
     uint32_t* cnt;
     uint32_t* cntp;
@@ -64,6 +65,7 @@
         *b = (uint8_t)((*b & 0xF0u) | id);
     } else ((uint8_t*)A.words)[4ull * sp] = (uint8_t)id;
 }
+#include "bp_masks.h"
 __device__ __forceinline__ uint32_t bp_lanes_below(unsigned long long m) {
     return (uint32_t)__builtin_amdgcn_mbcnt_hi((uint32_t)(m >> 32), __builtin_amdgcn_mbcnt_lo((uint32_t)m, 0u));
 }
@@ -111,7 +113,7 @@
     return t < max_blk ? t : max_blk;
 }
 __global__ __launch_bounds__(1024) void k_bp_segtab(const smc_dev_locus* __restrict__ loc, int n_loci, int n_seg, int seg_loci, uint32_t part, uint32_t max_blk,
-                                                    BpSeg* __restrict__ seg) {
+                                                    BpSeg* __restrict__ seg, uint32_t* __restrict__ n_live) {
     __shared__ uint32_t ws[4][16];
     __shared__ uint32_t carry[4];
     const int tid = threadIdx.x, lane = tid & 63, wid = tid >> 6;
@@ -148,7 +150,7 @@
             for (int w = 0; w < wid; ++w) pre += ws[c][w];
             ex[c] += pre;
         }
-        if (s < n_seg) { S.off = ex[0]; S.part_base = ex[1]; S.blk_base = ex[2]; S.cpart_base = ex[3]; seg[s] = S; }
+        if (s < n_seg) { S.off = ex[0]; S.part_base = ex[1]; S.blk_base = ex[2]; S.cpart_base = ex[3]; seg[s] = S; n_live[s] = v[0]; }
         __syncthreads();
         if (tid < 4) { uint32_t t = 0; for (int w = 0; w < 16; ++w) t += ws[tid][w]; carry[tid] += t; }
         __syncthreads();
@@ -291,7 +293,9 @@
 };
 template <int REG , int WAVES , bool BIG>
 __global__ __launch_bounds__(64 * WAVES) void k_bp_sort_seg(const BpSeg* __restrict__ seg, const uint2* __restrict__ k8 , int pair_bits, int passes,
-                                                      unsigned long long* k0, unsigned long long* k1, uint32_t* v0, uint32_t* v1, uint32_t only_above, uint32_t only_upto) {
+                                                      unsigned long long* k0, unsigned long long* k1, uint32_t* v0, uint32_t* v1, uint32_t only_above, uint32_t only_upto,
+                                                      const int32_t* __restrict__ kend , int start0,
+                                                      uint32_t* __restrict__ n_live ) {
     constexpr int LDS_MAX = 64 * WAVES * REG;
     if (!BIG && (seg[blockIdx.x].w1 - seg[blockIdx.x].w0) > only_upto) return;
     __shared__ uint32_t whist[WAVES][256];
@@ -301,45 +305,75 @@
     if (n == 0u || n > BP_LSORT_MAX || (BIG ? n <= only_above : false)) return;
     const int tid = threadIdx.x, lane = tid & 63, wid = tid >> 6;
     const uint32_t chunk = ((n + (uint32_t)WAVES - 1u) / (uint32_t)WAVES + 63u) & ~63u;
-    const uint32_t e0 = min(n, (uint32_t)wid * chunk), e1 = min(n, e0 + chunk);
+    uint32_t e0 = min(n, (uint32_t)wid * chunk), e1 = min(n, e0 + chunk);
     unsigned long long* kb[2] = {k0 + S.off, k1 + S.off};
     uint32_t* vb[2] = {v0 + S.off, v1 + S.off};
-    __shared__ uint32_t rng[4];
-    if (tid == 0) { rng[0] = 0xFFFFFFFFu; rng[1] = 0u; rng[2] = 0xFFFFFFFFu; rng[3] = 0u; }
-    __syncthreads();
+    const bool filter = n_live != nullptr;
+    const int p_first = start0 + (int)blockIdx.x * BP_TILE;
+    auto live = [&](uint32_t e) -> bool { return !filter || !bp_row_dead(kend[S.w0 + e], p_first); };
+    __shared__ uint32_t rng[5];
+    if (tid == 0) { rng[0] = 0xFFFFFFFFu; rng[1] = 0u; rng[2] = 0xFFFFFFFFu; rng[3] = 0u; rng[4] = 0u; }
+    __syncthreads();
+    const bool in_regs = n <= (uint32_t)LDS_MAX && chunk <= 64u * REG;
+    BpReg16 key, val;
+    uint32_t vm = 0u;
+#pragma unroll
+    for (int it = 0; it < 16; ++it) { key.at(it) = 0u; val.at(it) = 0u; }
     {
-        uint32_t b_lo = 0xFFFFFFFFu, b_hi = 0u, p_lo = 0xFFFFFFFFu, p_hi = 0u;
-        for (uint32_t e = e0 + (uint32_t)lane; e < e1; e += 64u) {
+        uint32_t b_lo = 0xFFFFFFFFu, b_hi = 0u, p_lo = 0xFFFFFFFFu, p_hi = 0u, nlv = 0u;
+        if (in_regs) {
+            if (e0 < e1) {
+                int ke[REG];
+#pragma unroll
+                for (int it = 0; it < REG; ++it) {
+                    const uint32_t a = S.w0 + min(e0 + 64u * (uint32_t)it + (uint32_t)lane, e1 - 1u);
+                    const uint2 kv = k8[a];
+                    key.at(it) = kv.x; val.at(it) = kv.y;
+                    ke[it] = filter ? kend[a] : 0x7FFFFFFF;
+                }
+#pragma unroll
+                for (int it = 0; it < REG; ++it) {
+                    const bool ok = e0 + 64u * (uint32_t)it + (uint32_t)lane < e1 && !bp_row_dead(ke[it], p_first);
+                    vm |= ok ? 1u << it : 0u;
+                    b_lo = min(b_lo, ok ? key.at(it) : 0xFFFFFFFFu); b_hi = max(b_hi, ok ? key.at(it) : 0u);
+                    p_lo = min(p_lo, ok ? val.at(it) : 0xFFFFFFFFu); p_hi = max(p_hi, ok ? val.at(it) : 0u);
+                }
+                nlv = (uint32_t)__popc(vm);
+            }
+        } else for (uint32_t e = e0 + (uint32_t)lane; e < e1; e += 64u) {
             const uint2 kv = k8[S.w0 + e];
+            if (!live(e)) continue;
             const uint32_t b = kv.x, q = kv.y;
             b_lo = min(b_lo, b); b_hi = max(b_hi, b); p_lo = min(p_lo, q); p_hi = max(p_hi, q);
+            ++nlv;
         }
         for (int o = 32; o; o >>= 1) {
             b_lo = min(b_lo, (uint32_t)__shfl_xor((int)b_lo, o)); b_hi = max(b_hi, (uint32_t)__shfl_xor((int)b_hi, o));
             p_lo = min(p_lo, (uint32_t)__shfl_xor((int)p_lo, o)); p_hi = max(p_hi, (uint32_t)__shfl_xor((int)p_hi, o));
-        }
-        if (lane == 0 && e0 < e1) { atomicMin(&rng[0], b_lo); atomicMax(&rng[1], b_hi); atomicMin(&rng[2], p_lo); atomicMax(&rng[3], p_hi); }
-    }
-    __syncthreads();
+            nlv += (uint32_t)__shfl_xor((int)nlv, o);
+        }
+        if (lane == 0 && nlv) { atomicMin(&rng[0], b_lo); atomicMax(&rng[1], b_hi); atomicMin(&rng[2], p_lo); atomicMax(&rng[3], p_hi); atomicAdd(&rng[4], nlv); }
+    }
+    __syncthreads();
+    const uint32_t nl = rng[4];
+    if (filter && tid == 0) n_live[blockIdx.x] = nl;
+    if (nl == 0u) return;
+    const uint32_t chunk2 = ((nl + (uint32_t)WAVES - 1u) / (uint32_t)WAVES + 63u) & ~63u;
+    const uint32_t f0 = min(nl, (uint32_t)wid * chunk2), f1 = min(nl, f0 + chunk2);
     const uint32_t bc_min = rng[0], pair_min = rng[2];
     const int pb = 32 - __builtin_clz((rng[3] - pair_min) | 1u), bb = 32 - __builtin_clz((rng[1] - bc_min) | 1u);
     int my_passes = (pb + bb + 7) / 8;
     if (pb + bb > 8 * passes) my_passes = passes;
     (void)pair_bits;
-    if (n <= (uint32_t)LDS_MAX && pb + bb <= 32 && chunk <= 64u * REG) {
+    if (in_regs && pb + bb <= 32) {
         __shared__ uint32_t lk[LDS_MAX];
         __shared__ uint16_t lv[LDS_MAX];
         static_assert(LDS_MAX <= 65536, "lv holds window indices in 16 bits");
-        BpReg16 key, val;
 #pragma unroll
         for (int it = 0; it < REG; ++it) {
-            const uint32_t e = e0 + 64u * (uint32_t)it + (uint32_t)lane;
-            key.at(it) = 0u; val.at(it) = 0u;
-            if (e < e1) {
-                val.at(it) = e;
-                const uint2 kv = k8[S.w0 + e];
-                key.at(it) = (kv.x - bc_min) << pb | (kv.y - pair_min);
-            }
+            const bool ok = (vm >> it) & 1u;
+            key.at(it) = ok ? (key.at(it) - bc_min) << pb | (val.at(it) - pair_min) : 0u;
+            val.at(it) = ok ? e0 + 64u * (uint32_t)it + (uint32_t)lane : 0u;
         }
         typedef __attribute__((address_space(1))) uint32_t glb_u32;
         glb_u32* const out = (glb_u32*)vb[passes & 1];
@@ -353,7 +387,7 @@
             __builtin_amdgcn_wave_barrier();
 #pragma unroll
             for (int it = 0; it < REG; ++it)
-                if (e0 + 64u * (uint32_t)it + (uint32_t)lane < e1) atomicAdd(&whist[wid][(key.at(it) >> shift) & dmask], 1u);
+                if ((vm >> it) & 1u) atomicAdd(&whist[wid][(key.at(it) >> shift) & dmask], 1u);
             __syncthreads();
             if (tid < 256) {
                 uint32_t run = 0;
@@ -376,7 +410,7 @@
 #pragma unroll
             for (int it = 0; it < REG; ++it) {
                 if (e0 + 64u * (uint32_t)it >= e1) break;
-                const bool valid = e0 + 64u * (uint32_t)it + (uint32_t)lane < e1;
+                const bool valid = (vm >> it) & 1u;
                 const uint32_t dgt = valid ? (key.at(it) >> shift) & dmask : 0u;
                 uint32_t rank, np;
                 bp_match(dgt, valid, dbits, rank, np);
@@ -392,10 +426,11 @@
             }
             if (last) break;
             __syncthreads();
+            e0 = f0; e1 = f1; vm = 0u;
 #pragma unroll
             for (int it = 0; it < REG; ++it) {
                 const uint32_t e = e0 + 64u * (uint32_t)it + (uint32_t)lane;
-                if (e < e1) { key.at(it) = lk[e]; val.at(it) = lv[e]; }
+                if (e < e1) { vm |= 1u << it; key.at(it) = lk[e]; val.at(it) = lv[e]; }
             }
             __syncthreads();
         }
@@ -408,20 +443,21 @@
         const uint32_t* vin = vb[ps & 1];
         unsigned long long* kout = kb[(ps & 1) ^ 1];
         uint32_t* vout = vb[(ps & 1) ^ 1];
-        auto fetch = [&](uint32_t e, unsigned long long& key, uint32_t& val) {
+        auto fetch = [&](uint32_t e, unsigned long long& key, uint32_t& val) -> bool {
             if (ps == 0) {
+                if (!live(e)) return false;
                 val = S.w0 + e;
                 const uint2 kv = k8[val];
                 key = ((unsigned long long)(kv.x - bc_min) << pb) | (unsigned long long)(kv.y - pair_min);
             } else { key = kin[e]; val = vin[e]; }
+            return true;
         };
 #pragma unroll
         for (int k = 0; k < 4; ++k) whist[wid][lane + 64 * k] = 0u;
         __builtin_amdgcn_wave_barrier();
         for (uint32_t e = e0 + (uint32_t)lane; e < e1; e += 64u) {
-            unsigned long long key; uint32_t val;
-            fetch(e, key, val);
-            atomicAdd(&whist[wid][(uint32_t)(key >> shift) & 255u], 1u);
+            unsigned long long key = 0; uint32_t val = 0;
+            if (fetch(e, key, val)) atomicAdd(&whist[wid][(uint32_t)(key >> shift) & 255u], 1u);
         }
         __syncthreads();
         if (tid < 256) {
@@ -444,10 +480,10 @@
         __syncthreads();
         for (uint32_t eb = e0; eb < e1; eb += 64u) {
             const uint32_t e = eb + (uint32_t)lane;
-            const bool valid = e < e1;
+            bool valid = e < e1;
             unsigned long long key = 0; uint32_t val = 0;
-            if (valid) fetch(e, key, val);
-            const uint32_t dgt = (uint32_t)(key >> shift) & 255u;
+            if (valid) valid = fetch(e, key, val);
+            const uint32_t dgt = valid ? (uint32_t)(key >> shift) & 255u : 0u;
             uint32_t rank, np;
             bp_match(dgt, valid, 8, rank, np);
             const uint32_t wo = valid ? whist[wid][dgt] : 0u;
@@ -457,6 +493,7 @@
             if (valid) { const uint32_t d = dbase[dgt] + wo + rank; kout[d] = key; vout[d] = val; }
         }
         __syncthreads();
+        e0 = f0; e1 = f1;
     }
 }
 
@@ -480,9 +517,7 @@
     W.p = A.start0 + W.l; W.p_first = A.start0 + l_first; W.p_last = A.start0 + l_last;
     W.a_lo = A.loc[l_first].w0; W.a_hi = A.loc[l_last].w1;
     W.seg_off = SG.off;
-    const uint32_t seg_end = SG.off + (SG.w1 - SG.w0);
-    W.j0 = SG.off + q * part;
-    W.j1 = min(seg_end, W.j0 + part);
+    bp_part_rows(SG.off, A.n_live[s], q, part, W.j0, W.j1);
     W.sub0 = SG.part_base + tis * SG.ppt + q * (part / (uint32_t)BP_SUB);
     {
         const uint32_t per = (uint32_t)A.part / (uint32_t)BP_SUB;
@@ -512,7 +547,6 @@
     v ^= (uint32_t)__builtin_amdgcn_update_dpp(0, (int)v, 0x143, 0xC, 0xF, false);
     return v;
 }
-#include "bp_masks.h"
 #define BP_MASK_LDS (66 + 32 + 32)
 struct BpCols { uint32_t C, NF, NB; };
 __device__ __forceinline__ BpCols bp_columns(uint32_t* lds, int lane, bool in_b, uint32_t rr, uint32_t nrows, int lo, int hi, uint32_t bc,
```

Result: faster. 80.94 million (median of 6 runs) (+1.5%).
